# LarsDoorenbos/ccdm-stochastic-segmentation

Hardware: AMD Instinct MI355X
Metric: segmentation samples/sec, LIDC 128x128 T=250 (higher is better)
Workload: dtype f32 (conv products as split fp16 hi/lo x3 on MFMA, fp32 accumulate)

## Files before the change

### ccdm_stochastic_segmentation_amd/csrc/ccdm_attn_block.hip

```cpp
#include "ccdm_common.h"
#include "ccdm_conv_common.h"

namespace ccdm {

struct AttnBlockK {
    ccdm_attn_block_args a;
    const float* wsq;
};

__device__ __forceinline__ void split8(const float* v, f16x8& hi, f16x8& lo) {
#pragma unroll
    for (int j = 0; j < 8; ++j) {
        hi[j] = (_Float16)v[j];
        lo[j] = (_Float16)(v[j] - (float)hi[j]);
    }
}
__device__ __forceinline__ void split4v(const float a, const float b, const float c, const float d, f16x4& hi, f16x4& lo) {
    hi[0] = (_Float16)a; hi[1] = (_Float16)b; hi[2] = (_Float16)c; hi[3] = (_Float16)d;
    lo[0] = (_Float16)(a - (float)hi[0]); lo[1] = (_Float16)(b - (float)hi[1]);
    lo[2] = (_Float16)(c - (float)hi[2]); lo[3] = (_Float16)(d - (float)hi[3]);
}
__device__ __forceinline__ f32x16 mfma3(const f16x8 ah, const f16x8 al, const f16x8 bh, const f16x8 bl, f32x16 acc) {
    acc = __builtin_amdgcn_mfma_f32_32x32x16_f16(al, bh, acc, 0, 0, 0);
    acc = __builtin_amdgcn_mfma_f32_32x32x16_f16(ah, bl, acc, 0, 0, 0);
// ... 171 lines not shown
#pragma unroll
        for (int u = 0; u < 2; ++u)
#pragma unroll
            for (int r = 0; r < 16; ++r) mx = fmaxf(mx, sc[u][r]);
        mx = fmaxf(mx, __shfl_xor(mx, 32));
        const float corr = __expf(m - mx);
        m = mx;
        l *= corr;
#pragma unroll
        for (int r = 0; r < 16; ++r) oo[r] *= corr;
#pragma unroll
        for (int u = 0; u < 2; ++u) {
            float p[16];
#pragma unroll
            for (int r = 0; r < 16; ++r) { p[r] = __expf(sc[u][r] - mx); l += p[r]; }
            const char* vr = vbase + qi * VROW + 2 * ((kt + u) * 32 + 4 * half);
#pragma unroll
            for (int s = 0; s < 2; ++s) {
                f16x8 ph, pl;
                split8(p + 8 * s, ph, pl);
                const f16x8 vh = cat4(*reinterpret_cast<const f16x4*>(vr + 32 * s), *reinterpret_cast<const f16x4*>(vr + 32 * s + 16));
                const f16x8 vl = cat4(*reinterpret_cast<const f16x4*>(vr + 2 * T + 32 * s), *reinterpret_cast<const f16x4*>(vr + 2 * T + 32 * s + 16));
                oo = mfma3(vh, vl, ph, pl, oo);
            }
        }
    }
    l += __shfl_xor(l, 32);
    const float inv = 1.0f / l;
    float* dst = a.out + ((size_t)n * T + mt * 32 + qi) * C + hd * 32 + 4 * half;
#pragma unroll
    for (int g4 = 0; g4 < 4; ++g4) {
        f32x4 v;
#pragma unroll
        for (int e = 0; e < 4; ++e) v[e] = oo[4 * g4 + e] * inv;
        *reinterpret_cast<f32x4*>(dst + 8 * g4) = v;
    }
}

template <int T, int C>
static int launch_one(const AttnBlockK& k, hipStream_t s) {
    using Geo = QkvAttnGeo<T, C>;
    static_assert(Geo::LDS <= 160 * 1024, "LDS budget");
    auto kern = k_qkv_attention<T, C>;
    static bool configured = false;
    if (!configured) {
        if (hipFuncSetAttribute(reinterpret_cast<const void*>(kern), hipFuncAttributeMaxDynamicSharedMemorySize, Geo::LDS) != hipSuccess)
            return fail("norm_qkv_attention: cannot reserve %d bytes of LDS", Geo::LDS);
        configured = true;
    }
    hipLaunchKernelGGL(kern, dim3(k.a.N, k.a.heads), dim3(Geo::NT), Geo::LDS, s, k);
    return 0;
}

bool attn_block_supported(int T, int C, int heads) {
    if (C != heads * 32) return false;
    return (T == 256 && (C == 96 || C == 128)) || (T == 64 && (C == 96 || C == 128)) || (T == 128 && (C == 128 || C == 256));
}

int launch_attn_block(const ccdm_attn_block_args& a, hipStream_t s) {
    CCDM_REQUIRE(a.x && a.out && a.stats && a.gamma && a.beta && a.wqkv && a.bqkv, "norm_qkv_attention: null pointer");
    CCDM_REQUIRE(a.N > 0 && a.slices >= 1, "norm_qkv_attention: N=%d slices=%d", a.N, a.slices);
    {
        int ntiles, NI;
        conv_ntiles(3 * a.C, &ntiles, &NI);
        CCDM_REQUIRE(ntiles == 3 * a.heads, "norm_qkv_attention: packed qkv weights have %d n-tiles, expected %d", ntiles, 3 * a.heads);
    }
    CCDM_REQUIRE(attn_block_supported(a.T, a.C, a.heads), "norm_qkv_attention: (T=%d, C=%d, heads=%d) is not built; use ccdm_conv2d (GN + qkv) + ccdm_attention",
                 a.T, a.C, a.heads);
    AttnBlockK k;
    k.a = a;
    k.wsq = reinterpret_cast<const float*>(static_cast<const char*>(a.wqkv) + (size_t)(a.C / 16) * (3 * a.C / 32) * 2048);
    int rc;
    if (a.T == 256 && a.C == 96) rc = launch_one<256, 96>(k, s);
    else if (a.T == 256) rc = launch_one<256, 128>(k, s);
    else if (a.T == 64 && a.C == 96) rc = launch_one<64, 96>(k, s);
    else if (a.T == 64) rc = launch_one<64, 128>(k, s);
    else if (a.C == 128) rc = launch_one<128, 128>(k, s);
    else rc = launch_one<128, 256>(k, s);
    if (rc) return rc;
    CCDM_CHECK_LAUNCH("norm_qkv_attention");
    return 0;
}

}

extern "C" int ccdm_norm_qkv_attention_supported(int T, int C, int heads) { return ccdm::attn_block_supported(T, C, heads) ? 1 : 0; }

extern "C" int ccdm_norm_qkv_attention(const ccdm_attn_block_args* a, void* stream) {
    if (!a) return ccdm::fail("ccdm_norm_qkv_attention: null args");
    return ccdm::launch_attn_block(*a, (hipStream_t)stream);
}
```

### ccdm_stochastic_segmentation_amd/csrc/ccdm_common.h

```cpp
#pragma once
#include <cstdlib>
#include <hip/hip_runtime.h>
#include <stdint.h>
#include <stdio.h>
#include <string>

#include "ccdm_hip.h"

namespace ccdm {

typedef float f32x16 __attribute__((ext_vector_type(16)));
typedef float f32x4 __attribute__((ext_vector_type(4)));
typedef _Float16 f16x8 __attribute__((ext_vector_type(8)));
typedef _Float16 f16x4 __attribute__((ext_vector_type(4)));

void set_error(const std::string& s);
int fail(const char* fmt, ...);

#define CCDM_CHECK_LAUNCH(what)                                               \
    do {                                                                      \
        hipError_t _e = hipGetLastError();                                    \
        if (_e != hipSuccess) return ::ccdm::fail("%s: %s", what, hipGetErrorString(_e)); \
    } while (0)

#define CCDM_REQUIRE(cond, ...)                     \
    do {                                            \
        if (!(cond)) return ::ccdm::fail(__VA_ARGS__); \
    } while (0)

static inline int cdiv(int a, int b) { return (a + b - 1) / b; }


#ifdef __HIPCC__
template <int BYTES>
__device__ __forceinline__ void warm_kernargs() {
    const auto kp = __builtin_amdgcn_kernarg_segment_ptr();
    static_assert(BYTES <= 512, "eight lines");
    constexpr int L = (BYTES + 63) / 64;
    unsigned d0, d1, d2, d3, d4, d5, d6, d7;
    asm volatile("s_load_dword %0, %8, %9\n\ts_load_dword %1, %8, %10\n\ts_load_dword %2, %8, %11\n\ts_load_dword %3, %8, %12\n\t"
                 "s_load_dword %4, %8, %13\n\ts_load_dword %5, %8, %14\n\ts_load_dword %6, %8, %15\n\ts_load_dword %7, %8, %16\n\t"
                 "s_waitcnt lgkmcnt(0)"
                 : "=&s"(d0), "=&s"(d1), "=&s"(d2), "=&s"(d3), "=&s"(d4), "=&s"(d5), "=&s"(d6), "=&s"(d7)
                 : "s"(kp), "i"(0), "i"(L > 1 ? 0x40 : 0), "i"(L > 2 ? 0x80 : 0), "i"(L > 3 ? 0xc0 : 0), "i"(L > 4 ? 0x100 : 0),
                   "i"(L > 5 ? 0x140 : 0), "i"(L > 6 ? 0x180 : 0), "i"(L > 7 ? 0x1c0 : 0));
}
#endif

struct ConvGeo {
    int TH, TW, waves, MI;
};
static inline ConvGeo conv_geo(int Hout, int Wout, int stride, bool up2 = false, bool fine = false) {
    if (up2) return Wout >= 16 ? ConvGeo{8, 16, 4, 1} : ConvGeo{8, 8, 2, 1};
    if (stride == 2) return Wout >= 16 ? ConvGeo{8, 16, 4, 1} : ConvGeo{8, 8, 2, 1};
    const int area = Hout * Wout;
    if (fine && area <= 1024) return Wout >= 16 && area > 256 ? ConvGeo{8, 16, 4, 1} : ConvGeo{8, 8, 2, 1};
    if (Wout >= 32 && area > 512) return {8, 32, 4, 2};
    if (Wout >= 16 && area > 128) return {8, 16, 4, 1};
    return {8, 8, 2, 1};
}
static inline void conv_ntiles(int Cout, int* ntiles_padded, int* NI) {
    int raw = cdiv(Cout, 32);
    if (raw <= 4) { *NI = raw; *ntiles_padded = raw; return; }
    for (int ni = 4; ni >= 2; --ni)
        if (raw % ni == 0) { *NI = ni; *ntiles_padded = raw; return; }
    *NI = 4; *ntiles_padded = cdiv(raw, 4) * 4;
}
static inline int conv_cin_pad(int Cin) { return cdiv(Cin, 32) * 32; }

int launch_conv(const ccdm_conv_args& a, hipStream_t s);
int launch_conv_input_absmax(const ccdm_conv_args& a, float* out, hipStream_t s);
int launch_attention(const float* qkv, float* out, int N, int T, int Ta, int C, int heads, int order, hipStream_t s);
int launch_posterior(const ccdm_post_args& a, hipStream_t s);
int launch_stats_fold(const double* in, int N, int S_in, int C, int S_out, double* out, hipStream_t s);
int launch_attn_block(const ccdm_attn_block_args& a, hipStream_t s);
int launch_resample(const ccdm_resample_args& a, hipStream_t s);
int launch_stem(const ccdm_stem_args& a, hipStream_t s);
int launch_head(const ccdm_head_args& a, const ccdm_post_args& post, hipStream_t s);
bool attn_block_supported(int T, int C, int heads);

}
```

### ccdm_stochastic_segmentation_amd/csrc/ccdm_conv.hip

```cpp
#include "ccdm_common.h"
#include "ccdm_conv_common.h"

#include <cmath>
#include <cstdlib>
#include <type_traits>
#include <vector>

namespace ccdm {


constexpr int min_waves(int mi, int ni, int prec, int ckt, int threads) {
    if (threads > 512) return 3;
    if (prec != CCDM_PREC_F32 && ckt >= 32) return 2;
    return mi * ni <= 2 ? 3 : (mi * ni <= 4 ? 2 : 1);
}

template <int PREC, int CKT, int KS, int STRIDE, int TH, int TW, int WAVES, int MI, int NI, int KSP = 1, bool UP2 = false, bool SKWT = false>
__global__ __launch_bounds__(WAVES * KSP * 64, min_waves(MI, NI, PREC, CKT, WAVES * KSP * 64)) void k_conv(const ConvK k) {
    constexpr int NT = WAVES * KSP * 64;
    static_assert(KSP == 1 || KSP == KS, "tap split is by kernel row");
    static_assert(!UP2 || (KS == 3 && STRIDE == 1 && KSP == 1 && (NI == 1 || NI == 4) && PREC != CCDM_PREC_F32), "sub-pixel form: 3x3, stride 1, F16X3, one phase or all four");
    constexpr int NTAP = UP2 ? 4 : KS * KS;
    constexpr int CK = CKT, PIXB = conv_pixb(PREC, CKT);
    constexpr int KST = CK / 16;
// ... 852 lines not shown
    ConvK k;
    k.a = a;
    k.core_unmasked = 0;
    const int prec = a.prec & 255;
    k.cin_pad = cin_pad_for(C, prec);
    k.cin_pad_skip = a.skip0 ? cin_pad_for(a.SC0 + a.SC1, prec) : 0;
    k.skip_wide = 0;
    int NI;
    conv_ntiles(up2 ? 4 * a.Cout : a.Cout, &k.ntiles, &NI);
    const int tH = up2 ? a.Hin : a.Hout, tW = up2 ? a.Win : a.Wout;
    const ConvGeo g = conv_geo(tH, tW, a.stride, up2, a.fine_slices != 0);
    if (up2) NI = g.TW == 16 ? 4 : 1;
    else if (g.TW < 32) NI = 1;
    else {
        const long blocks2 = (long)a.N * conv_slices(a.Hout, a.Wout, a.stride, false, a.fine_slices) * (k.ntiles / 2);
        NI = (k.ntiles % 2 == 0 && blocks2 >= 512) ? 2 : 1;
    }
    k.tiles_x = cdiv(tW, g.TW);
    k.tiles_y = cdiv(tH, g.TH);
    k.slices = conv_slices(tH, tW, a.stride, up2, a.fine_slices);
    const bool ks = conv_takes_ks(a);
    if (ks) k.slices = conv_ks_slices(a);
    k.wscale = reinterpret_cast<const float*>(static_cast<const char*>(a.w) +
                                              (up2 ? packed_frag_bytes(4 * a.Cout, C, 2, prec) : packed_frag_bytes(a.Cout, C, a.ksize, prec)));
    const int want_slices = (up2 && NI == 1 ? 4 : 1) * k.slices;
    if (a.out_stats) CCDM_REQUIRE(a.out_slices == want_slices, "conv: out_slices %d != %d", a.out_slices, want_slices);
    if (up2 && upconv_eligible(a)) {
        const int rcu = launch_upconv(a, k.slices, k.ntiles, k.wscale, s);
        if (rcu) return rcu;
        CCDM_CHECK_LAUNCH("upconv");
        return 0;
    }
    if (conv1x1_eligible(a, k.slices)) {
        const int rc1 = launch_conv1x1(a, k.slices, k.ntiles, k.wscale, s);
        if (rc1) return rc1;
        CCDM_CHECK_LAUNCH("conv1x1");
        return 0;
    }
    if (ks) {
        const int rck = launch_conv_ks(a, k.ntiles, k.wscale, s);
        if (rck) return rck;
        CCDM_CHECK_LAUNCH("conv_ks");
        return 0;
    }
    const int HP = ((g.TH - 1) * a.stride + a.ksize) * ((g.TW - 1) * a.stride + a.ksize);
    const int ck = chunk_ck(a, g);
    {
        k.skip_wide = (a.skip0 && prec == CCDM_PREC_F16X3 && a.ksize == 3 && a.stride == 1 && !a.up && g.TW == 32 && NI == 1 && ck == 16 &&
                       a.SC0 % 32 == 0 && a.SC1 % 32 == 0 && !(a.prec >> 8)) ? 1 : 0;
    }
    {
        const int SC = a.SC0 + a.SC1;
        const bool chan_ok = a.C0 % ck == 0 && a.C1 % ck == 0 && (!a.skip0 || (a.SC0 % ck == 0 && a.SC1 % ck == 0 && SC > 0));
        k.core_unmasked = ((up2 ? a.Win : Wc) % (g.TW * a.stride) == 0 && chan_ok) ? 1 : 0;
    }
    CCDM_REQUIRE(a.C1 == 0 || a.C0 % ck == 0, "conv: first source has %d channels; a concatenated input must split at a multiple of the %d-channel chunk", a.C0, ck);
    CCDM_REQUIRE(a.SC1 == 0 || a.SC0 % ck == 0, "conv: first skip source has %d channels; a concatenated input must split at a multiple of the %d-channel chunk", a.SC0, ck);
    CCDM_REQUIRE((k.cin_pad + k.cin_pad_skip) / ck <= 64, "conv: %d input (+%d skip) channels make more than 64 chunks of %d (chunk descriptors live in the 64 lanes of a register)",
                 k.cin_pad, k.cin_pad_skip, ck);
    size_t lds = (size_t)HP * conv_pixb(prec, ck);
    lds = (lds + 15) / 16 * 16;
    if (prec != CCDM_PREC_F32) lds += (size_t)(up2 ? 4 : a.ksize * a.ksize) * (ck / 16) * NI * FRAG_BYTES;
    const int ksp = tap_split(a, g) ? 3 : 1;
    const size_t red = (size_t)g.waves * ksp * NI * 32 * 16;
    if (lds < red) lds = red;
    const size_t epi = (size_t)g.waves * ksp * g.MI * 32 * EPI_ROW * 4;
    if (lds < epi) lds = epi;
    if (a.stats0) {
        const size_t nthreads = (size_t)g.waves * ksp * 64;
        const size_t ex = (size_t)C > nthreads ? (size_t)C : nthreads;
        if (lds < ex * 16) lds = ex * 16;
        lds += (size_t)C * 8;
    }
    CCDM_REQUIRE(lds <= 160 * 1024, "conv: LDS %zu too large", lds);
    dim3 grid(a.N * k.slices, k.ntiles / NI);
    const int rc = prec == CCDM_PREC_F32 ? launch_prec<CCDM_PREC_F32>(k, g, NI, ck, grid, lds, s)
                   : prec == CCDM_PREC_F16 ? launch_prec<CCDM_PREC_F16>(k, g, NI, ck, grid, lds, s)
                                           : launch_prec<CCDM_PREC_F16X3>(k, g, NI, ck, grid, lds, s);
    if (rc) return rc;
    CCDM_CHECK_LAUNCH("conv");
    return 0;
}

}

extern "C" int ccdm_conv_slices(int Hout, int Wout, int stride, int ksize) {
    (void)ksize;
    return ccdm::conv_slices(Hout, Wout, stride);
}

extern "C" int ccdm_upconv_supported(int Cin, int Cout, int prec) {
    return prec == CCDM_PREC_F16X3 && Cin > 0 && Cin % 4 == 0 && Cout > 0 && Cout % 32 == 0;
}

extern "C" int ccdm_upconv_slices(int Hin, int Win) {
    return ccdm::upconv_out_slices(Hin, Win, 0);
}

extern "C" int ccdm_conv_out_slices(const ccdm_conv_args* a) {
    if (!a) return ccdm::fail("ccdm_conv_out_slices: null args");
    return ccdm::conv_out_slices(*a);
}

extern "C" int ccdm_conv_slices_ex(int Hin, int Win, int ksize, int stride, int up, int fine) {
    if (up == 2) return ccdm::upconv_out_slices(Hin, Win, fine);
    const int Hc = up ? 2 * Hin : Hin, Wc = up ? 2 * Win : Win, pad = ksize / 2;
    return ccdm::conv_slices((Hc + 2 * pad - ksize) / stride + 1, (Wc + 2 * pad - ksize) / stride + 1, stride, false, fine);
}

extern "C" int ccdm_conv2d(const ccdm_conv_args* a, void* stream) {
    if (!a) return ccdm::fail("ccdm_conv2d: null args");
    return ccdm::launch_conv(*a, (hipStream_t)stream);
}

extern "C" size_t ccdm_pack_conv_weight_ex(const float* oihw, int Cout, int Cin, int ksize, int prec, const float* cout_absmax, void* out);

extern "C" size_t ccdm_pack_conv_weight(const float* oihw, int Cout, int Cin, int ksize, int prec, void* out) {
    return ccdm_pack_conv_weight_ex(oihw, Cout, Cin, ksize, prec, nullptr, out);
}

extern "C" size_t ccdm_pack_conv_weight_ex(const float* oihw, int Cout, int Cin, int ksize, int prec, const float* cout_absmax, void* out) {
    if (prec != CCDM_PREC_F32 && prec != CCDM_PREC_F16X3) { ccdm::fail("pack: precision %d not built", prec); return 0; }
    int ntiles, NI;
    ccdm::conv_ntiles(Cout, &ntiles, &NI);
    const int cin_pad = ccdm::cin_pad_for(Cin, prec), taps = ksize * ksize;
    const size_t frag = ccdm::packed_frag_bytes(Cout, Cin, ksize, prec);
    const size_t total = frag + (prec == CCDM_PREC_F16X3 ? (size_t)ntiles * 32 * sizeof(float) : 0);
    if (!out) return total;
    if (prec == CCDM_PREC_F32) {
        float* o = static_cast<float*>(out);
        for (int tap = 0; tap < taps; ++tap)
            for (int kp = 0; kp < cin_pad / 2; ++kp)
                for (int nt = 0; nt < ntiles; ++nt)
                    for (int l = 0; l < 64; ++l) {
                        const int co = nt * 32 + (l & 31), ci = 2 * kp + (l >> 5);
                        float v = 0.f;
                        if (co < Cout && ci < Cin) v = oihw[((size_t)co * Cin + ci) * taps + tap];
                        o[(((size_t)tap * (cin_pad / 2) + kp) * ntiles + nt) * 64 + l] = v;
                    }
        return total;
    }
    _Float16* o = static_cast<_Float16*>(out);
    float* sc = reinterpret_cast<float*>(static_cast<char*>(out) + frag);
    std::vector<float> mul(ntiles * 32, 1.0f);
    for (int co = 0; co < ntiles * 32; ++co) {
        float mx = 0.f;
        if (co < Cout) {
            if (cout_absmax) mx = cout_absmax[co];
            else for (size_t i = 0; i < (size_t)Cin * taps; ++i) mx = fmaxf(mx, fabsf(oihw[(size_t)co * Cin * taps + i]));
        }
        int e = 0;
        if (mx > 0.f && std::isfinite(mx)) { int ex; frexpf(mx, &ex); e = 10 - ex; }
        if (e > 60) e = 60;
        if (e < -60) e = -60;
        mul[co] = ldexpf(1.0f, e);
        sc[co] = ldexpf(1.0f, -e) / ccdm::ACT_PRESCALE;
    }
    for (int tap = 0; tap < taps; ++tap)
        for (int ks = 0; ks < cin_pad / 16; ++ks)
            for (int nt = 0; nt < ntiles; ++nt)
                for (int l = 0; l < 64; ++l)
                    for (int j = 0; j < 8; ++j) {
                        const int co = nt * 32 + (l & 31), ci = 16 * ks + 8 * (l >> 5) + j;
                        float v = 0.f;
                        if (co < Cout && ci < Cin) v = oihw[((size_t)co * Cin + ci) * taps + tap] * mul[co];
                        const _Float16 hi = (_Float16)v;
// ... 28 lines not shown
```

### ccdm_stochastic_segmentation_amd/csrc/ccdm_engine.hip

```cpp
#include "ccdm_common.h"

#include <map>
#include <vector>

namespace ccdm {

__global__ void k_step_set(int32_t* p, int32_t v) { *p = v; }
__global__ void k_step_inc(int32_t* p) { *p += 1; }
__global__ void k_run_set(ccdm_post_run* dst, const ccdm_post_run v) { *dst = v; }
__global__ __launch_bounds__(256) void k_absmax(const float* __restrict__ x, size_t n4, float* out) {
    float m = 0.f;
    bool bad = false;
    for (size_t i = (size_t)blockIdx.x * blockDim.x + threadIdx.x; i < n4; i += (size_t)gridDim.x * blockDim.x) {
        const float4 v = reinterpret_cast<const float4*>(x)[i];
        bad |= !(fabsf(v.x) <= 3.0e38f) | !(fabsf(v.y) <= 3.0e38f) | !(fabsf(v.z) <= 3.0e38f) | !(fabsf(v.w) <= 3.0e38f);
        m = fmaxf(m, fmaxf(fmaxf(fabsf(v.x), fabsf(v.y)), fmaxf(fabsf(v.z), fabsf(v.w))));
    }
    if (bad) m = __builtin_inff();
#pragma unroll
    for (int off = 32; off > 0; off >>= 1) m = fmaxf(m, __shfl_xor(m, off));
    if ((threadIdx.x & 63) == 0) atomicMax(reinterpret_cast<unsigned*>(out), __float_as_uint(m));
}

struct Op {
    int kind;
    ccdm_conv_args conv;
    const float* qkv; float* out; int N, T, C, heads, order;
    const double* fin; double* fout; int S_in, S_out;
    ccdm_attn_block_args ab;
    ccdm_resample_args rs;
    ccdm_stem_args st;
    ccdm_head_args hd;
};

static int launch_op(const Op& op, hipStream_t s) {
    switch (op.kind) {
        case 6: return fail("engine: the head + epilogue op is launched with the epilogue's arguments");
        case 0: return launch_conv(op.conv, s);
        case 1: return launch_attention(op.qkv, op.out, op.N, op.T, op.T, op.C, op.heads, op.order, s);
        case 2: return launch_stats_fold(op.fin, op.N, op.S_in, op.C, op.S_out, op.fout, s);
        case 3: return launch_attn_block(op.ab, s);
        case 4: return launch_resample(op.rs, s);
        default: return launch_stem(op.st, s);
    }
}

}

struct ccdm_engine {
    int32_t* step = nullptr;
    std::vector<ccdm::Op> ops;
    ccdm_post_args post{};
    bool has_post = false;
    ccdm_post_run run{};
    ccdm_post_run* run_dev = nullptr;
    bool run_dirty = false;
    int next_row = 0;
    hipGraph_t graph = nullptr;
    hipGraphExec_t exec = nullptr;
    bool graph_valid = false;
    int graph_with_epilogue = -1;
    int captures = 0;
    struct Tap { std::vector<hipEvent_t> ev; int n = 0; };
    std::map<int, Tap> taps;
};

using namespace ccdm;

static void drop_graph(ccdm_engine* e) {
    if (e->exec) { (void)hipGraphExecDestroy(e->exec); e->exec = nullptr; }
    if (e->graph) { (void)hipGraphDestroy(e->graph); e->graph = nullptr; }
    e->graph_valid = false;
}

static int launch_step(ccdm_engine* e, int with_epilogue, hipStream_t s, bool profile) {
    for (size_t i = 0; i < e->ops.size(); ++i) {
        const Op& op = e->ops[i];
        ccdm_engine::Tap* tp = nullptr;
        if (profile) {
            auto it = e->taps.find((int)i);
            if (it != e->taps.end() && (size_t)(2 * it->second.n + 1) < it->second.ev.size()) tp = &it->second;
        }
        if (tp) (void)hipEventRecord(tp->ev[2 * tp->n], s);
        int rc;
        if (op.kind == 6) {
            rc = (with_epilogue && e->has_post) ? launch_head(op.hd, e->post, s) : fail("engine_run: this step ends in a fused head + epilogue op: with_epilogue must be 1 and an epilogue set");
        } else rc = launch_op(op, s);
        if (tp) { (void)hipEventRecord(tp->ev[2 * tp->n + 1], s); tp->n++; }
        if (rc) return rc;
    }
    if (with_epilogue && e->has_post && !(e->ops.size() && e->ops.back().kind == 6)) {
        int rc = launch_posterior(e->post, s);
        if (rc) return rc;
    }
    hipLaunchKernelGGL(k_step_inc, dim3(1), dim3(1), 0, s, e->step);
    CCDM_CHECK_LAUNCH("step_inc");
    return 0;
}

extern "C" ccdm_engine* ccdm_engine_create(int32_t* step_counter) {
    if (!step_counter) { fail("engine_create: null step counter"); return nullptr; }
    ccdm_engine* e = new ccdm_engine();
    e->step = step_counter;
    return e;
}

extern "C" void ccdm_engine_destroy(ccdm_engine* e) {
    if (!e) return;
    drop_graph(e);
    for (auto& kv : e->taps)
        for (hipEvent_t ev : kv.second.ev) (void)hipEventDestroy(ev);
    delete e;
}

extern "C" int ccdm_engine_add_conv(ccdm_engine* e, const ccdm_conv_args* a) {
    CCDM_REQUIRE(e && a, "engine_add_conv: null");
    Op op{};
    op.kind = 0;
    op.conv = *a;
    op.conv.step_ptr = e->step;
    e->ops.push_back(op);
    drop_graph(e);
    return (int)e->ops.size() - 1;
}

extern "C" int ccdm_engine_add_attention(ccdm_engine* e, const float* qkv, float* out, int N, int T, int C, int heads, int order) {
    CCDM_REQUIRE(e && qkv && out, "engine_add_attention: null");
    Op op{};
    op.kind = 1;
    op.qkv = qkv; op.out = out; op.N = N; op.T = T; op.C = C; op.heads = heads; op.order = order;
    e->ops.push_back(op);
    drop_graph(e);
    return (int)e->ops.size() - 1;
}

extern "C" int ccdm_engine_add_norm_qkv_attention(ccdm_engine* e, const ccdm_attn_block_args* a) {
    CCDM_REQUIRE(e && a, "engine_add_norm_qkv_attention: null");
    CCDM_REQUIRE(attn_block_supported(a->T, a->C, a->heads), "engine_add_norm_qkv_attention: (T=%d, C=%d, heads=%d) is not built", a->T, a->C, a->heads);
    Op op{};
    op.kind = 3;
    op.ab = *a;
    e->ops.push_back(op);
    drop_graph(e);
    return (int)e->ops.size() - 1;
}

extern "C" int ccdm_engine_add_stats_fold(ccdm_engine* e, const double* in, int N, int S_in, int C, int S_out, double* out) {
    CCDM_REQUIRE(e && in && out, "engine_add_stats_fold: null");
    Op op{};
    op.kind = 2;
    op.fin = in; op.fout = out; op.N = N; op.S_in = S_in; op.C = C; op.S_out = S_out;
    e->ops.push_back(op);
    drop_graph(e);
    return (int)e->ops.size() - 1;
}

extern "C" int ccdm_engine_add_resample(ccdm_engine* e, const ccdm_resample_args* a) {
    CCDM_REQUIRE(e && a, "engine_add_resample: null");
    Op op{};
    op.kind = 4;
    op.rs = *a;
    e->ops.push_back(op);
    drop_graph(e);
    return (int)e->ops.size() - 1;
}

extern "C" int ccdm_engine_add_stem(ccdm_engine* e, const ccdm_stem_args* a) {
    CCDM_REQUIRE(e && a, "engine_add_stem: null");
    CCDM_REQUIRE(ccdm_stem_conv_supported(a->Cs, a->Cout, a->H, a->W, CCDM_PREC_F16X3), "engine_add_stem: Cs=%d Cout=%d %dx%d is not built", a->Cs, a->Cout, a->H, a->W);
    Op op{};
    op.kind = 5;
    op.st = *a;
    e->ops.push_back(op);
    drop_graph(e);
    return (int)e->ops.size() - 1;
}

extern "C" int ccdm_engine_add_head_posterior(ccdm_engine* e, const ccdm_head_args* a) {
    CCDM_REQUIRE(e && a, "engine_add_head_posterior: null");
    CCDM_REQUIRE(ccdm_head_posterior_supported(a->C, a->K, a->H, a->W, CCDM_PREC_F16X3), "engine_add_head_posterior: C=%d K=%d %dx%d is not built", a->C, a->K, a->H, a->W);
    Op op{};
    op.kind = 6;
    op.hd = *a;
    e->ops.push_back(op);
    drop_graph(e);
    return (int)e->ops.size() - 1;
}

extern "C" int ccdm_engine_set_epilogue(ccdm_engine* e, const ccdm_post_args* a) {
    CCDM_REQUIRE(e && a, "engine_set_epilogue: null");
    e->post = *a;
    e->post.step_ptr = e->step;
    e->has_post = true;
    if (e->run_dev) {
        e->post.run = e->run_dev;
        const ccdm_post_args& p = e->post;
        e->run = ccdm_post_run{p.noise, p.noise_step_stride, p.philox_seed, p.sample_offset, p.noise_row0, p.out_probs, p.out_onehot, p.posterior_out};
        e->run_dirty = true;
    }
    drop_graph(e);
    return 0;
}

extern "C" int ccdm_engine_num_ops(const ccdm_engine* e) { return e ? (int)e->ops.size() : -1; }
extern "C" int ccdm_engine_num_captures(const ccdm_engine* e) { return e ? e->captures : -1; }

extern "C" int ccdm_engine_set_run_block(ccdm_engine* e, void* dev_block) {
    CCDM_REQUIRE(e && e->has_post, "engine_set_run_block: no epilogue set");
    CCDM_REQUIRE(dev_block && (reinterpret_cast<uintptr_t>(dev_block) & 7) == 0, "engine_set_run_block: null or misaligned block");
    e->run_dev = static_cast<ccdm_post_run*>(dev_block);
    e->post.run = e->run_dev;
    const ccdm_post_args& p = e->post;
    e->run = ccdm_post_run{p.noise, p.noise_step_stride, p.philox_seed, p.sample_offset, p.noise_row0, p.out_probs, p.out_onehot, p.posterior_out};
    e->run_dirty = true;
    drop_graph(e);
    return 0;
}

extern "C" int ccdm_engine_set_run(ccdm_engine* e, const float* noise, int64_t noise_step_stride, int32_t noise_row0, uint64_t philox_seed,
                                   uint32_t sample_offset, float* out_probs, int64_t* out_onehot, float* posterior_out) {
    CCDM_REQUIRE(e && e->has_post, "engine_set_run: no epilogue set");
    if (e->run_dev) {
        const ccdm_post_run r{noise, noise_step_stride, philox_seed, sample_offset, noise_row0, out_probs, out_onehot, posterior_out};
        const ccdm_post_run& o = e->run;
        const bool same = o.noise == r.noise && o.noise_step_stride == r.noise_step_stride && o.philox_seed == r.philox_seed &&
                          o.sample_offset == r.sample_offset && o.noise_row0 == r.noise_row0 && o.out_probs == r.out_probs &&
                          o.out_onehot == r.out_onehot && o.posterior_out == r.posterior_out;
        if (!same) { e->run = r; e->run_dirty = true; }
        return 0;
    }
    ccdm_post_args& p = e->post;
    const bool same = p.noise == noise && p.noise_step_stride == noise_step_stride && p.noise_row0 == noise_row0 && p.philox_seed == philox_seed &&
                      p.sample_offset == sample_offset && p.out_probs == out_probs && p.out_onehot == out_onehot &&
                      p.posterior_out == posterior_out;
    if (!same) drop_graph(e);
    p.noise = noise; p.noise_step_stride = noise_step_stride; p.noise_row0 = noise_row0; p.philox_seed = philox_seed; p.sample_offset = sample_offset;
    p.out_probs = out_probs; p.out_onehot = out_onehot; p.posterior_out = posterior_out;
    return 0;
}

extern "C" int ccdm_engine_run(ccdm_engine* e, int first_row, int n_steps, int with_epilogue, int use_graph, void* stream) {
    CCDM_REQUIRE(e, "engine_run: null engine");
    CCDM_REQUIRE(n_steps >= 0, "engine_run: n_steps=%d", n_steps);
    hipStream_t s = (hipStream_t)stream;
    hipLaunchKernelGGL(k_step_set, dim3(1), dim3(1), 0, s, e->step, (int32_t)first_row);
    CCDM_CHECK_LAUNCH("step_set");
    e->next_row = first_row + n_steps;
    if (e->run_dev && e->run_dirty) {
        hipLaunchKernelGGL(k_run_set, dim3(1), dim3(1), 0, s, e->run_dev, e->run);
        CCDM_CHECK_LAUNCH("run_set");
        e->run_dirty = false;
    }
    const bool profile = !e->taps.empty();
    if (profile) {
        use_graph = 0;
        if (first_row == 0) for (auto& kv : e->taps) kv.second.n = 0;
    }
    if (use_graph) {
        if (!e->graph_valid || e->graph_with_epilogue != with_epilogue) {
            drop_graph(e);
            hipError_t err = hipStreamBeginCapture(s, hipStreamCaptureModeRelaxed);
            if (err != hipSuccess) return fail("engine_run: BeginCapture: %s", hipGetErrorString(err));
            const int rc = launch_step(e, with_epilogue, s, false);
            err = hipStreamEndCapture(s, &e->graph);
            if (rc) { if (e->graph) { (void)hipGraphDestroy(e->graph); e->graph = nullptr; } return rc; }
            if (err != hipSuccess) return fail("engine_run: EndCapture: %s", hipGetErrorString(err));
            err = hipGraphInstantiate(&e->exec, e->graph, nullptr, nullptr, 0);
            if (err != hipSuccess) return fail("engine_run: GraphInstantiate: %s", hipGetErrorString(err));
            e->graph_valid = true;
            e->graph_with_epilogue = with_epilogue;
            e->captures++;
        }
        for (int i = 0; i < n_steps; ++i) {
            hipError_t err = hipGraphLaunch(e->exec, s);
            if (err != hipSuccess) return fail("engine_run: GraphLaunch: %s", hipGetErrorString(err));
        }
        return 0;
    }
    for (int i = 0; i < n_steps; ++i) {
        int rc = launch_step(e, with_epilogue, s, profile);
        if (rc) return rc;
    }
    return 0;
}

extern "C" int ccdm_engine_profile_op(ccdm_engine* e, int op_index, int capacity) {
    CCDM_REQUIRE(e, "engine_profile_op: null engine");
    if (op_index < 0) {
        for (auto& kv : e->taps)
            for (hipEvent_t ev : kv.second.ev) (void)hipEventDestroy(ev);
        e->taps.clear();
        return 0;
    }
    CCDM_REQUIRE(op_index < (int)e->ops.size(), "engine_profile_op: op %d out of range", op_index);
    ccdm_engine::Tap& t = e->taps[op_index];
    t.n = 0;
    while ((int)t.ev.size() < 2 * capacity) {
        hipEvent_t ev;
        if (hipEventCreate(&ev) != hipSuccess) return fail("engine_profile_op: hipEventCreate failed");
        t.ev.push_back(ev);
    }
    return 0;
}

extern "C" int ccdm_engine_profile_read(ccdm_engine* e, int op_index, double* mean_ms, double* min_ms, double* max_ms) {
    CCDM_REQUIRE(e, "engine_profile_read: null engine");
    auto it = e->taps.find(op_index);
    CCDM_REQUIRE(it != e->taps.end(), "engine_profile_read: op %d is not tapped", op_index);
    ccdm_engine::Tap& t = it->second;
    double sum = 0, mn = 1e30, mx = 0;
    int n = 0;
    for (int i = 0; i < t.n; ++i) {
        float ms = 0.f;
        if (hipEventSynchronize(t.ev[2 * i + 1]) != hipSuccess) continue;
        if (hipEventElapsedTime(&ms, t.ev[2 * i], t.ev[2 * i + 1]) != hipSuccess) continue;
        sum += ms; if (ms < mn) mn = ms; if (ms > mx) mx = ms; ++n;
    }
    if (mean_ms) *mean_ms = n ? sum / n : 0.0;
    if (min_ms) *min_ms = n ? mn : 0.0;
    if (max_ms) *max_ms = n ? mx : 0.0;
    return n;
}

extern "C" int ccdm_engine_input_absmax(ccdm_engine* e, float* out, int row, void* stream) {
    CCDM_REQUIRE(e && out, "engine_input_absmax: null");
    hipStream_t s = (hipStream_t)stream;
    const int r = row >= 0 ? row : (e->next_row > 0 ? e->next_row - 1 : 0);
    hipLaunchKernelGGL(k_step_set, dim3(1), dim3(1), 0, s, e->step, (int32_t)r);
    CCDM_CHECK_LAUNCH("step_set");
    int rc = 0;
    for (size_t i = 0; i < e->ops.size() && !rc; ++i) {
        const Op& op = e->ops[i];
        if (op.kind == 0) rc = launch_conv_input_absmax(op.conv, out + i, s);
        else if (op.kind == 6) {
            ccdm_conv_args c{};
            c.in0 = op.hd.x; c.C0 = op.hd.C; c.stats0 = op.hd.stats; c.slices0 = op.hd.slices; c.gamma = op.hd.gamma; c.beta = op.hd.beta;
            c.eps = op.hd.eps; c.act = CCDM_ACT_SILU; c.N = op.hd.N; c.Hin = c.Hout = op.hd.H; c.Win = c.Wout = op.hd.W; c.ksize = 3; c.stride = 1;
            c.emb_off = -1; c.prec = CCDM_PREC_F16X3;
            rc = launch_conv_input_absmax(c, out + i, s);
        }
        else if (op.kind == 5 || op.kind == 1) {
            const size_t n4 = op.kind == 5 ? (size_t)op.st.N * op.st.H * op.st.W * op.st.Cs / 4 : (size_t)op.N * op.T * 3 * op.C / 4;
            const float* src = op.kind == 5 ? op.st.xin : op.qkv;
            const unsigned bx = (unsigned)(n4 / 256 < 1 ? 1 : (n4 / 256 > 1024 ? 1024 : n4 / 256));
            hipLaunchKernelGGL(k_absmax, dim3(bx), dim3(256), 0, s, src, n4, out + i);
            if (hipGetLastError() != hipSuccess) rc = fail("engine_input_absmax: attention operand probe failed to launch");
        }
    }
    hipLaunchKernelGGL(k_step_set, dim3(1), dim3(1), 0, s, e->step, (int32_t)e->next_row);
    CCDM_CHECK_LAUNCH("step_set");
    return rc;
}

extern "C" int ccdm_engine_describe_op(const ccdm_engine* e, int i, char* buf, int buflen) {
    CCDM_REQUIRE(e && buf && buflen > 0, "engine_describe_op: bad args");
    CCDM_REQUIRE(i >= 0 && i < (int)e->ops.size(), "engine_describe_op: op %d out of range", i);
    const Op& op = e->ops[i];
    if (op.kind == 0) {
        const ccdm_conv_args& a = op.conv;
        snprintf(buf, buflen, "conv%dx%d %d%s->%d in%dx%d out%dx%d s%d%s%s%s%s%s%s", a.ksize, a.ksize, a.C0 + a.C1,
                 a.C1 ? "(cat)" : "", a.Cout, a.Hin, a.Win, a.Hout, a.Wout, a.stride, a.up ? " up2x" : "",
                 a.stats0 ? " gn" : "", a.act ? " silu" : "", a.emb_off >= 0 ? " +emb" : "", a.resid ? " +res" : "",
                 a.out_stats ? " stats" : "");
    } else if (op.kind == 1) {
        snprintf(buf, buflen, "attention T=%d C=%d heads=%d order=%d", op.T, op.C, op.heads, op.order);
// ... 15 lines not shown
```

### ccdm_stochastic_segmentation_amd/csrc/ccdm_misc.hip

```cpp
#include "ccdm_common.h"

#include <stdarg.h>

namespace ccdm {

static thread_local std::string g_err;
void set_error(const std::string& s) { g_err = s; }
int fail(const char* fmt, ...) {
    char buf[512];
    va_list ap;
    va_start(ap, fmt);
    vsnprintf(buf, sizeof buf, fmt, ap);
    va_end(ap);
    g_err = buf;
    return -1;
}

__global__ void k_gn_stats(const float* __restrict__ x, int HW, int C, int slices, double* __restrict__ stats) {
    extern __shared__ __attribute__((aligned(16))) char smem[];
    double* red = reinterpret_cast<double*>(smem);
    const int Q = C >> 2, R = blockDim.x / Q;
    const int q = threadIdx.x % Q, r = threadIdx.x / Q;
    const int s = blockIdx.x, n = blockIdx.y;
    const int p0 = (int)((long long)HW * s / slices), p1 = (int)((long long)HW * (s + 1) / slices);
// ... 48 lines not shown
    float m = -INFINITY, l = 0.f;

    for (int j0 = 0; j0 < T; j0 += 64) {
        __syncthreads();
        for (int item = lane; item < 64 * (D / 4); item += 64) {
            const int row = item / (D / 4), c4 = item % (D / 4);
            float4 kv = make_float4(0, 0, 0, 0), vv = make_float4(0, 0, 0, 0);
            if (j0 + row < T) {
                const float* p = base + (size_t)(j0 + row) * C3;
                kv = *reinterpret_cast<const float4*>(p + koff + 4 * c4);
                vv = *reinterpret_cast<const float4*>(p + voff + 4 * c4);
            }
            kv.x *= scale; kv.y *= scale; kv.z *= scale; kv.w *= scale;
            *reinterpret_cast<float4*>(kt + row * D + 4 * c4) = kv;
            *reinterpret_cast<float4*>(vt + row * D + 4 * c4) = vv;
        }
        __syncthreads();
        const int jn = (T - j0) < 64 ? (T - j0) : 64;
        for (int jb = 0; jb < jn; jb += 16) {
            float s[16];
            float mx = m;
#pragma unroll
            for (int jj = 0; jj < 16; ++jj) {
                const float* kr = kt + (jb + jj) * D;
                float acc = 0.f;
#pragma unroll
                for (int c = 0; c < D; ++c) acc = fmaf(q[c], kr[c], acc);
                s[jj] = (jb + jj < jn) ? acc : -INFINITY;
                mx = fmaxf(mx, s[jj]);
            }
            const float corr = expf(m - mx);
            l *= corr;
#pragma unroll
            for (int c = 0; c < D; ++c) o[c] *= corr;
            m = mx;
#pragma unroll
            for (int jj = 0; jj < 16; ++jj) {
                const float p = expf(s[jj] - mx);
                l += p;
                const float* vr = vt + (jb + jj) * D;
#pragma unroll
                for (int c = 0; c < D; ++c) o[c] = fmaf(p, vr[c], o[c]);
            }
        }
    }
    if (t < T) {
        const float inv = 1.0f / l;
        float* dst = out + ((size_t)n * Ta + t) * C + h * D;
#pragma unroll
        for (int c = 0; c < D; c += 4)
            *reinterpret_cast<float4*>(dst + c) = make_float4(o[c] * inv, o[c + 1] * inv, o[c + 2] * inv, o[c + 3] * inv);
    }
}

int launch_attention_mfma(const float* qkv, float* out, int N, int T, int Ta, int C, int heads, int order, hipStream_t s);
int attention_mfma_width(int D);

int launch_attention(const float* qkv, float* out, int N, int T, int Ta, int C, int heads, int order, hipStream_t s) {
    CCDM_REQUIRE(qkv && out, "attention: null pointer");
    CCDM_REQUIRE(heads > 0 && C % heads == 0, "attention: C=%d not divisible by heads=%d", C, heads);
    CCDM_REQUIRE(T > 0 && Ta >= T, "attention: T=%d, %d rows allocated per sample", T, Ta);
    const int D = C / heads;
    const bool force_valu = (order & CCDM_ATTENTION_FORCE_VALU) != 0;
    order &= 255;
    const bool mfma_ok = attention_mfma_width(D) > 0 && !(D == 32 && (T % 32 != 0 || Ta != T));
    if (mfma_ok && !force_valu) return launch_attention_mfma(qkv, out, N, T, Ta, C, heads, order, s);
    dim3 grid(cdiv(T, 64), heads, N), block(64);
    switch (D) {
        case 4: hipLaunchKernelGGL(k_attention<4>, grid, block, 0, s, qkv, out, T, Ta, C, heads, order); break;
        case 8: hipLaunchKernelGGL(k_attention<8>, grid, block, 0, s, qkv, out, T, Ta, C, heads, order); break;
        case 12: hipLaunchKernelGGL(k_attention<12>, grid, block, 0, s, qkv, out, T, Ta, C, heads, order); break;
        case 16: hipLaunchKernelGGL(k_attention<16>, grid, block, 0, s, qkv, out, T, Ta, C, heads, order); break;
        case 24: hipLaunchKernelGGL(k_attention<24>, grid, block, 0, s, qkv, out, T, Ta, C, heads, order); break;
        case 32: hipLaunchKernelGGL(k_attention<32>, grid, block, 0, s, qkv, out, T, Ta, C, heads, order); break;
        case 48: hipLaunchKernelGGL(k_attention<48>, grid, block, 0, s, qkv, out, T, Ta, C, heads, order); break;
        case 64: hipLaunchKernelGGL(k_attention<64>, grid, block, 0, s, qkv, out, T, Ta, C, heads, order); break;
        default: return fail("attention: head width %d (C=%d / heads=%d) is built neither on the matrix cores (multiples of 4 up to 128) nor "
                             "on the vector path (4, 8, 12, 16, 24, 32, 48, 64): choose num_heads / num_head_channels accordingly", D, C, heads);
    }
    CCDM_CHECK_LAUNCH("attention");
    return 0;
}

__device__ __forceinline__ float silu_t(float x) { return x / (1.0f + expf(-x)); }

__global__ void k_time_table(const float* __restrict__ sinus, int mc,
                             const float* __restrict__ w0, const float* __restrict__ b0,
                             const float* __restrict__ w2, const float* __restrict__ b2,
                             const float* __restrict__ wcat, const float* __restrict__ bcat, int E,
                             float* __restrict__ emb_out, float* __restrict__ out) {
    extern __shared__ __attribute__((aligned(16))) float sm[];
    const int ted = 4 * mc;
    float* x = sm;
    float* h1 = sm + mc;
    float* e = h1 + ted;
    const int s = blockIdx.x;
    for (int i = threadIdx.x; i < mc; i += blockDim.x) x[i] = sinus[(size_t)s * mc + i];
    __syncthreads();
    for (int j = threadIdx.x; j < ted; j += blockDim.x) {
        float acc = 0.f;
        for (int i = 0; i < mc; ++i) acc = fmaf(w0[(size_t)j * mc + i], x[i], acc);
        h1[j] = silu_t(acc + b0[j]);
    }
    __syncthreads();
    for (int j = threadIdx.x; j < ted; j += blockDim.x) {
        float acc = 0.f;
        for (int i = 0; i < ted; ++i) acc = fmaf(w2[(size_t)j * ted + i], h1[i], acc);
        const float v = acc + b2[j];
        if (emb_out) emb_out[(size_t)s * ted + j] = v;
        e[j] = silu_t(v);
    }
    __syncthreads();
    for (int j = threadIdx.x; j < E; j += blockDim.x) {
        float acc = 0.f;
        for (int i = 0; i < ted; ++i) acc = fmaf(wcat[(size_t)j * ted + i], e[i], acc);
        out[(size_t)s * E + j] = acc + bcat[j];
    }
}

__global__ void k_nchw_to_nhwc(const float* __restrict__ src, float* __restrict__ dst, int C, int HW,
                               int dst_stride, int dst_off, size_t total) {
    const size_t i = (size_t)blockIdx.x * blockDim.x + threadIdx.x;
    if (i >= total) return;
    const int p = (int)(i % HW);
    const size_t nc = i / HW;
    const int c = (int)(nc % C);
    const size_t n = nc / C;
    dst[(n * HW + p) * dst_stride + dst_off + c] = src[i];
}

__global__ void k_onehot_to_xin(const uint8_t* __restrict__ idx, float* __restrict__ xin, int K, int stride, size_t npix) {
    const size_t i = (size_t)blockIdx.x * blockDim.x + threadIdx.x;
    if (i >= npix) return;
    const int k = idx[i];
    float* d = xin + i * stride;
    for (int c = 0; c < K; ++c) d[c] = (c == k) ? 1.0f : 0.0f;
}

}

using namespace ccdm;

extern "C" int ccdm_version(void) { return CCDM_ABI_VERSION; }
extern "C" const char* ccdm_last_error_string(void) { return g_err.c_str(); }

namespace ccdm {
__global__ void k_stats_fold(const double* __restrict__ in, int S_in, int C2, int S_out, double* __restrict__ out) {
    const int n = blockIdx.y;
    const int i = blockIdx.x * blockDim.x + threadIdx.x;
    if (i >= S_out * C2) return;
    const int j = i / C2, c = i % C2;
    const int s0 = (int)((long long)j * S_in / S_out), s1 = (int)((long long)(j + 1) * S_in / S_out);
    const double* p = in + (size_t)n * S_in * C2 + c;
    double t = 0.0;
    for (int s = s0; s < s1; s += 16) {
        double v[16];
#pragma unroll
        for (int u = 0; u < 16; ++u) v[u] = p[(size_t)min(s + u, s1 - 1) * C2];
#pragma unroll
        for (int u = 0; u < 16; ++u) t += s + u < s1 ? v[u] : 0.0;
    }
    out[(size_t)n * S_out * C2 + i] = t;
}
int launch_stats_fold(const double* in, int N, int S_in, int C, int S_out, double* out, hipStream_t s) {
    CCDM_REQUIRE(in && out && N > 0 && C > 0, "stats_fold: bad arguments");
    CCDM_REQUIRE(S_out >= 1 && S_out <= CCDM_STATS_MAX_SLICES && S_in >= S_out, "stats_fold: %d -> %d slices", S_in, S_out);
    dim3 grid((unsigned)cdiv(S_out * C * 2, 256), (unsigned)N);
    hipLaunchKernelGGL(k_stats_fold, grid, dim3(256), 0, s, in, S_in, 2 * C, S_out, out);
    CCDM_CHECK_LAUNCH("stats_fold");
    return 0;
}
}

extern "C" int ccdm_stats_fold(const double* in, int N, int S_in, int C, int S_out, double* out, void* stream) {
    return ccdm::launch_stats_fold(in, N, S_in, C, S_out, out, (hipStream_t)stream);
}

extern "C" int ccdm_gn_stats(const float* x, int N, int HW, int C, int slices, double* stats, void* stream) {
    CCDM_REQUIRE(x && stats, "gn_stats: null pointer");
    CCDM_REQUIRE(C % 4 == 0 && C >= 4 && C <= 1024, "gn_stats: C=%d must be a multiple of 4 in [4,1024]", C);
    CCDM_REQUIRE(slices >= 1 && slices <= CCDM_STATS_MAX_SLICES, "gn_stats: slices=%d", slices);
    const int Q = C / 4;
    const int R = 256 / Q > 0 ? 256 / Q : 1;
    dim3 grid(slices, N), block(Q * R);
    const size_t lds = (size_t)Q * R * 8 * sizeof(double);
    hipLaunchKernelGGL(k_gn_stats, grid, block, lds, (hipStream_t)stream, x, HW, C, slices, stats);
    CCDM_CHECK_LAUNCH("gn_stats");
    return 0;
}

extern "C" int ccdm_attention(const float* qkv, float* out, int N, int T, int C, int heads, int order, void* stream) {
    return launch_attention(qkv, out, N, T, T, C, heads, order, (hipStream_t)stream);
}

extern "C" int ccdm_time_table(const float* sinus, int S, int mc, const float* w0, const float* b0,
                               const float* w2, const float* b2, const float* wcat, const float* bcat, int E,
                               float* emb_out, float* out, void* stream) {
    CCDM_REQUIRE(sinus && w0 && b0 && w2 && b2 && out, "time_table: null pointer");
    CCDM_REQUIRE(E == 0 || (wcat && bcat), "time_table: null wcat/bcat");
    CCDM_REQUIRE(mc > 0 && mc <= 1024, "time_table: model_channels=%d", mc);
    if (S <= 0) return 0;
    const size_t lds = (size_t)(mc + 8 * mc) * sizeof(float);
    hipLaunchKernelGGL(k_time_table, dim3(S), dim3(256), lds, (hipStream_t)stream, sinus, mc, w0, b0, w2, b2,
                       wcat, bcat, E, emb_out, out);
    CCDM_CHECK_LAUNCH("time_table");
    return 0;
}

extern "C" int ccdm_nchw_to_nhwc(const float* src, float* dst, int N, int C, int HW, int dst_stride, int dst_off, void* stream) {
    CCDM_REQUIRE(src && dst, "nchw_to_nhwc: null pointer");
    const size_t total = (size_t)N * C * HW;
    if (!total) return 0;
    hipLaunchKernelGGL(k_nchw_to_nhwc, dim3((unsigned)((total + 255) / 256)), dim3(256), 0, (hipStream_t)stream,
                       src, dst, C, HW, dst_stride, dst_off, total);
    CCDM_CHECK_LAUNCH("nchw_to_nhwc");
    return 0;
}

extern "C" int ccdm_onehot_to_xin(const uint8_t* idx, float* xin, int N, int HW, int K, int xin_stride, void* stream) {
    CCDM_REQUIRE(idx && xin, "onehot_to_xin: null pointer");
    const size_t npix = (size_t)N * HW;
    if (!npix) return 0;
    hipLaunchKernelGGL(k_onehot_to_xin, dim3((unsigned)((npix + 255) / 256)), dim3(256), 0, (hipStream_t)stream,
                       idx, xin, K, xin_stride, npix);
    CCDM_CHECK_LAUNCH("onehot_to_xin");
    return 0;
}


namespace ccdm {

constexpr int LN_MAX_PER_LANE = 24;
__global__ __launch_bounds__(256) void k_layernorm(const float* __restrict__ x, const float* __restrict__ gamma, const float* __restrict__ beta,
                                                   float eps, long rows, int C, float* __restrict__ out) {
    const long row = (long)blockIdx.x * 4 + (threadIdx.x >> 6);
    const int lane = threadIdx.x & 63;
    if (row >= rows) return;
    const float* xr = x + row * C;
    float v[LN_MAX_PER_LANE];
    float sum = 0.f;
#pragma unroll
    for (int i = 0; i < LN_MAX_PER_LANE; ++i) {
        const int c = lane + 64 * i;
        v[i] = c < C ? xr[c] : 0.f;
        sum += v[i];
    }
#pragma unroll
    for (int off = 32; off > 0; off >>= 1) sum += __shfl_xor(sum, off);
    const float mean = sum / (float)C;
    float dsum = 0.f;
#pragma unroll
    for (int i = 0; i < LN_MAX_PER_LANE; ++i) {
        const int c = lane + 64 * i;
// ... 122 lines not shown
```

### ccdm_stochastic_segmentation_amd/csrc/ccdm_resample.hip

```cpp
#include "ccdm_common.h"
#include "ccdm_conv_common.h"

namespace ccdm {

struct ResampleK {
    ccdm_conv_args g;
    float* out_act;
    float* out_raw;
    int mode;
};

__device__ __forceinline__ float4 resample_act(const float4 v, const float2* ab, const int c, const bool has_gn, const bool silu) {
    float x[4] = {v.x, v.y, v.z, v.w};
#pragma unroll
    for (int j = 0; j < 4; ++j) {
        float y = x[j];
        if (has_gn) y = fmaf(y, ab[c + j].x, ab[c + j].y);
        if (silu) y = y / (1.0f + expf(-y));
        x[j] = y;
    }
    return make_float4(x[0], x[1], x[2], x[3]);
}

__device__ __forceinline__ float4 pool4(const float4 a, const float4 b, const float4 c, const float4 d) {
    return make_float4((((a.x + b.x) + c.x) + d.x) * 0.25f, (((a.y + b.y) + c.y) + d.y) * 0.25f,
                       (((a.z + b.z) + c.z) + d.z) * 0.25f, (((a.w + b.w) + c.w) + d.w) * 0.25f);
}

__global__ __launch_bounds__(256) void k_resample(const ResampleK k) {
    extern __shared__ __attribute__((aligned(16))) char smem_rs[];
    float2* ab = reinterpret_cast<float2*>(smem_rs);
    const ccdm_conv_args& a = k.g;
    const int n = blockIdx.y, C = a.C0, Q = C >> 2;
    const bool has_gn = a.stats0 != nullptr && k.out_act != nullptr, silu = a.act == CCDM_ACT_SILU;
    if (has_gn) {
        compute_gn_affine(a, n, 0, ab);
        __syncthreads();
    }
    const int Ho = a.Hout, Wo = a.Wout;
    const float* in = a.in0 + (size_t)n * a.Hin * a.Win * C;
    float* oa = k.out_act ? k.out_act + (size_t)n * Ho * Wo * C : nullptr;
    float* orw = k.out_raw ? k.out_raw + (size_t)n * Ho * Wo * C : nullptr;
    const long long items = (long long)Ho * Wo * Q;
    for (long long item = (long long)blockIdx.x * blockDim.x + threadIdx.x; item < items; item += (long long)gridDim.x * blockDim.x) {
        const int q = (int)(item % Q), p = (int)(item / Q), ox = p % Wo, oy = p / Wo, c = 4 * q;
        const size_t o = (size_t)p * C + c;
        if (k.mode == CCDM_RESAMPLE_AVGPOOL2) {
            const float* r0 = in + ((size_t)(2 * oy) * a.Win + 2 * ox) * C + c;
            const float* r1 = r0 + (size_t)a.Win * C;
            const float4 v00 = *reinterpret_cast<const float4*>(r0), v01 = *reinterpret_cast<const float4*>(r0 + C);
            const float4 v10 = *reinterpret_cast<const float4*>(r1), v11 = *reinterpret_cast<const float4*>(r1 + C);
            if (orw) *reinterpret_cast<float4*>(orw + o) = pool4(v00, v01, v10, v11);
            if (oa)
                *reinterpret_cast<float4*>(oa + o) = pool4(resample_act(v00, ab, c, has_gn, silu), resample_act(v01, ab, c, has_gn, silu),
                                                           resample_act(v10, ab, c, has_gn, silu), resample_act(v11, ab, c, has_gn, silu));
        } else {
            const float4 v = *reinterpret_cast<const float4*>(in + ((size_t)(oy >> 1) * a.Win + (ox >> 1)) * C + c);
            if (orw) *reinterpret_cast<float4*>(orw + o) = v;
            if (oa) *reinterpret_cast<float4*>(oa + o) = resample_act(v, ab, c, has_gn, silu);
        }
    }
}

int launch_resample(const ccdm_resample_args& r, hipStream_t s) {
    CCDM_REQUIRE(r.in && (r.out_act || r.out_raw), "resample: null pointer");
    CCDM_REQUIRE(r.mode == CCDM_RESAMPLE_AVGPOOL2 || r.mode == CCDM_RESAMPLE_NEAREST_UP2, "resample: mode = %d", r.mode);
    CCDM_REQUIRE(r.C > 0 && r.C % 4 == 0 && r.N > 0 && r.Hin > 0 && r.Win > 0, "resample: N=%d C=%d %dx%d", r.N, r.C, r.Hin, r.Win);
    CCDM_REQUIRE(r.act == CCDM_ACT_NONE || r.act == CCDM_ACT_SILU, "resample: act = %d", r.act);
    ResampleK k{};
    k.g.in0 = r.in; k.g.C0 = r.C;
    k.g.N = r.N; k.g.Hin = r.Hin; k.g.Win = r.Win;
    k.g.Hout = r.mode == CCDM_RESAMPLE_AVGPOOL2 ? r.Hin / 2 : 2 * r.Hin;
    k.g.Wout = r.mode == CCDM_RESAMPLE_AVGPOOL2 ? r.Win / 2 : 2 * r.Win;
    CCDM_REQUIRE(k.g.Hout > 0 && k.g.Wout > 0, "resample: AvgPool2d(2) of a %dx%d image is empty", r.Hin, r.Win);
    k.g.act = r.act; k.g.eps = r.eps; k.g.emb_off = -1;
    if (r.stats) {
        CCDM_REQUIRE(r.out_act, "resample: GroupNorm statistics without an out_act destination");
        CCDM_REQUIRE(r.C % 32 == 0 && r.C <= CCDM_MAX_CHANNELS, "resample: GroupNorm(32, %d)", r.C);
        CCDM_REQUIRE(r.gamma && r.beta && r.slices >= 1 && r.slices <= CCDM_STATS_MAX_SLICES, "resample: GroupNorm needs gamma/beta and 1..%d slices (got %d)",
                     CCDM_STATS_MAX_SLICES, r.slices);
        k.g.stats0 = r.stats; k.g.slices0 = r.slices; k.g.gamma = r.gamma; k.g.beta = r.beta;
    }
    k.out_act = r.out_act; k.out_raw = r.out_raw; k.mode = r.mode;
    const long long items = (long long)k.g.Hout * k.g.Wout * (r.C / 4);
    const long long want = (items + 1023) / 1024;
    const int bx = (int)(want < 1 ? 1 : (want > 64 ? 64 : want));
    hipLaunchKernelGGL(k_resample, dim3(bx, r.N), dim3(256), r.stats ? (size_t)r.C * 8 : 0, s, k);
    CCDM_CHECK_LAUNCH("resample");
    return 0;
}

}

extern "C" int ccdm_resample(const ccdm_resample_args* a, void* stream) {
    if (!a) return ccdm::fail("ccdm_resample: null args");
    return ccdm::launch_resample(*a, (hipStream_t)stream);
}
```

### ccdm_stochastic_segmentation_amd/engine.py

```python
from __future__ import annotations

import ctypes as C
import math
from dataclasses import dataclass
from typing import Dict, List, Optional, Sequence, Tuple

import numpy as np
import torch

from . import hip
from .unet_spec import GN_EPS, UNetSpec


@dataclass
class DevTensor:
    buf: torch.Tensor
    C: int
    h: int
    w: int
    stats: Optional[torch.Tensor] = None
    slices: int = 0

    @property
    def ptr(self) -> int:
        return self.buf.data_ptr()

    @property
    def stats_ptr(self) -> int:
        return self.stats.data_ptr() if self.stats is not None else 0


def timestep_embedding_host(timesteps: torch.Tensor, dim: int, max_period: int = 10000) -> torch.Tensor:
    half = dim // 2
    freqs = torch.exp(-math.log(max_period) * torch.arange(start=0, end=half, dtype=torch.float32) / half)
    args = timesteps[:, None].float() * freqs[None]
    emb = torch.cat([torch.cos(args), torch.sin(args)], dim=-1)
    if dim % 2:
        emb = torch.cat([emb, torch.zeros_like(emb[:, :1])], dim=-1)
    return emb


class TileCanvas:

    def __init__(self, n: int, Hc: int, Wc: int, sy: int, sx: int, K: int, device: torch.device):
        self.n, self.Hc, self.Wc, self.sy, self.sx = int(n), int(Hc), int(Wc), int(sy), int(sx)
        self.xt = torch.zeros((self.n, self.Hc * self.Wc), dtype=torch.uint8, device=device)
        self.out_probs = torch.empty((self.n, self.Hc, self.Wc, K), dtype=torch.float32, device=device)
        self.out_onehot = torch.empty((self.n, self.Hc, self.Wc, K), dtype=torch.int64, device=device)


class SamplerEngine:

    def __init__(self, spec: UNetSpec, state_dict: Dict[str, torch.Tensor], N: int, H: int, W: int,
                 num_classes: int, img_channels: int, device: torch.device, max_steps: int,
                 feature_shape: Optional[Tuple[int, int, int]] = None, prec: int = hip.PREC_F32, fine_slices: int = 0,
                 f32_layers=frozenset()):
        self.lib = hip.load()
        self.f32_layers = frozenset(f32_layers)
        self.fine_slices = int(fine_slices)
        if device.type != "cuda":
            raise hip.CcdmHipError("SamplerEngine needs a HIP device (torch device 'cuda'); there is no CPU path")
        self.spec, self.N, self.H, self.W = spec, int(N), int(H), int(W)
        self.K, self.C_img = int(num_classes), int(img_channels)
        self.device, self.prec = device, prec
        self.max_steps = max(int(max_steps), self.N, 1)
        if spec.in_channels != self.K + self.C_img or spec.out_channels != self.K:
            raise ValueError("spec channels do not match num_classes/img_channels")
        self._keep: List[torch.Tensor] = []
        self._sd = {k: v.detach().to("cpu", torch.float32).contiguous() for k, v in state_dict.items()}
        self.feature_shape = feature_shape
        self._handle = None
        self._tile_canvas: Optional[TileCanvas] = None
        self._tile_canvas_key = None
        self._bound_xt: Optional[torch.Tensor] = None
        self._bound_ws: Optional[torch.Tensor] = None
        self._slot_pools: Optional[Tuple[torch.Tensor, torch.Tensor]] = None
        with torch.cuda.device(device):
            self.stream = torch.cuda.Stream(device=device)
            with torch.cuda.stream(self.stream):
                self._build()
            self.stream.synchronize()

    def _dev(self, shape, dtype=torch.float32, zero=False) -> torch.Tensor:
        t = (torch.zeros if zero else torch.empty)(shape, dtype=dtype, device=self.device)
        self._keep.append(t)
        return t

    def _upload(self, arr) -> torch.Tensor:
        t = torch.as_tensor(np.ascontiguousarray(arr)) if not isinstance(arr, torch.Tensor) else arr.contiguous()
        d = t.to(self.device)
        self._keep.append(d)
        return d

    def _act(self, C_: int, h: int, w: int, stats: bool, slices: int = 0) -> DevTensor:
        buf = self._dev((self.N, h, w, C_))
        t = DevTensor(buf, C_, h, w)
        if stats:
            t.slices = slices
            t.stats = self._dev((self.N, t.slices, C_, 2), torch.float64)
        return t

    def _fold_stats(self, t: DevTensor) -> None:
        if t.stats is None or t.slices <= hip.STATS_MAX_SLICES:
            return
        folded = self._dev((self.N, hip.STATS_FOLD_SLICES, t.C, 2), torch.float64)
        hip.check(self.lib.ccdm_engine_add_stats_fold(self._handle, t.stats.data_ptr(), self.N, t.slices, t.C, hip.STATS_FOLD_SLICES,
                                                      folded.data_ptr()), "engine_add_stats_fold")
        self.op_names.append("stats_fold")
        self.op_info.append(dict(kind="stats_fold", name="stats_fold", io_bytes=0, gn_read_bytes=0, weight_bytes=0, flop=0))
        t.stats, t.slices = folded, hip.STATS_FOLD_SLICES

    def _conv(self, src: Sequence[DevTensor], wkey: str, cout: int, ksize: int, *, gn: Optional[str] = None,
              act: int = hip.ACT_NONE, stride: int = 1, up: bool = False, emb_off: int = -1,
              film_off: int = -1, resid: Optional[DevTensor] = None, stats: bool = True,
              skip_src: Optional[Sequence[DevTensor]] = None, skip_key: Optional[str] = None) -> DevTensor:
        sd = self._sd
        prec = hip.PREC_F32 if wkey in self.f32_layers else self.prec
        pack_prec = hip.PREC_F16X3 if prec == hip.PREC_F16 else prec
        a, b = src[0], (src[1] if len(src) > 1 else None)
        cin = a.C + (b.C if b else 0)
        w = sd[wkey + ".weight"].numpy()
        assert w.shape[0] == cout and w.shape[1] <= cin, (wkey, w.shape, cin, cout)
        if w.shape[1] < cin:
            wp = np.zeros((cout, cin) + tuple(w.shape[2:]), np.float32)
            wp[:, : w.shape[1]] = w
            w = wp
        bias_np = sd[wkey + ".bias"].numpy()
        absmax = None
        if skip_src is not None:
            ws = sd[skip_key + ".weight"].numpy().reshape(cout, -1)
            absmax = np.maximum(np.abs(w.reshape(cout, -1)).max(1), np.abs(ws).max(1)).astype(np.float32)
            skip_w = self._upload(hip.pack_conv_weight(ws.reshape(cout, -1, 1, 1), 1, pack_prec, absmax))
            bias_np = bias_np + sd[skip_key + ".bias"].numpy()
        subpixel = bool(up) and ksize == 3 and stride == 1 and resid is None and skip_src is None and gn is None and emb_off < 0 and \
            bool(self.lib.ccdm_upconv_supported(cin, cout, prec))
        wdev = self._upload(hip.pack_upconv_weight(w, prec) if subpixel else hip.pack_conv_weight(w, ksize, pack_prec, absmax))
        bias = self._upload(bias_np)
        hin, win = a.h, a.w
        hc, wc = (2 * hin, 2 * win) if up else (hin, win)
        pad = ksize // 2
# ... 203 lines not shown
        ted, mc = spec.time_embed_dim, spec.model_channels
        self.emb_offsets: Dict[str, int] = {}
        ws, bs, off = [], [], 0
        for name, l in spec.all_layers():
            if l.kind == "res":
                self.emb_offsets[name] = off
                ws.append(sd[name + ".emb_layers.1.weight"].numpy())
                bs.append(sd[name + ".emb_layers.1.bias"].numpy())
                off += ws[-1].shape[0]
        self.E = off
        self.wcat = self._upload(np.concatenate(ws, 0))
        self.bcat = self._upload(np.concatenate(bs, 0))
        self.te = [self._upload(sd[k].numpy()) for k in
                   ("time_embed.0.weight", "time_embed.0.bias", "time_embed.2.weight", "time_embed.2.bias")]
        S = self.max_steps
        self.sinus = self._dev((S, mc))
        self.emb_table = self._dev((S, self.E))
        self.step_table = self._dev((S, 4), zero=True)

        self.Cs = (K + self.C_img + 3) // 4 * 4
        self.xt = self._dev((N, H * W), torch.uint8, zero=True)
        self.xin = DevTensor(self._dev((N, H, W, self.Cs), zero=True), self.Cs, H, W)
        self.feat: Optional[DevTensor] = None
        if spec.feature_condition_idx:
            if self.feature_shape is None:
                raise ValueError("this model concatenates feature conditioning; feature_shape=(C,h,w) is required")
            fc, fh, fw = self.feature_shape
            if fc != spec.feature_channels:
                raise ValueError(f"feature_condition has {fc} channels, model expects {spec.feature_channels}")
            self.feat = DevTensor(self._dev((N, fh, fw, fc)), fc, fh, fw,
                                  self._dev((N, 1, fc, 2), torch.float64), 1)
        self.out_probs = self._dev((N, H, W, K))
        self.out_onehot = self._dev((N, H, W, K), torch.int64)

        hs: List[DevTensor] = []
        h = self.xin
        for i, blk in enumerate(spec.input_blocks):
            src = [h]
            if i in spec.feature_condition_idx:
                if (self.feat.h, self.feat.w) != (h.h, h.w):
                    raise ValueError(f"feature_condition is {self.feat.h}x{self.feat.w}, U-Net stage is {h.h}x{h.w}")
                src = [h, self.feat]
            h = self._layers(blk, src)
            hs.append(h)
        h = self._layers(spec.middle_block, [h])
        for blk in spec.output_blocks:
            h = self._layers(blk, [h, hs.pop()])
        Kp = (K + 3) // 4 * 4
        if Kp != K:
            wk, bk = self._sd["out.2.weight"], self._sd["out.2.bias"]
            self._sd["out.2.weight"] = torch.cat([wk, torch.zeros((Kp - K,) + tuple(wk.shape[1:]))], 0)
            self._sd["out.2.bias"] = torch.cat([bk, torch.zeros(Kp - K)], 0)
        self.head_fused = bool(self.prec == hip.PREC_F16X3 and "out.2" not in self.f32_layers and not self.fine_slices and h.stats is not None
                               and lib.ccdm_head_posterior_supported(h.C, K, H, W, hip.PREC_F16X3))
        self._head_src = h
        self.head = None if self.head_fused else self._conv([h], "out.2", Kp, 3, gn="out.0", act=hip.ACT_SILU, stats=False)
        self.head_ce: Optional[DevTensor] = None
        if spec.ce_head:
            Kc = K - 1
            Kcp = (Kc + 3) // 4 * 4
            if Kcp != Kc:
                wk, bk = self._sd["out_ce.2.weight"], self._sd["out_ce.2.bias"]
                self._sd["out_ce.2.weight"] = torch.cat([wk, torch.zeros((Kcp - Kc,) + tuple(wk.shape[1:]))], 0)
                self._sd["out_ce.2.bias"] = torch.cat([bk, torch.zeros(Kcp - Kc)], 0)
            self.head_ce = self._conv([h], "out_ce.2", Kcp, 3, gn="out_ce.0", act=hip.ACT_SILU, stats=False)
        if self.head_fused:
            sdw = self._sd
            a = hip.HeadArgs()
            a.x, a.stats, a.slices = h.ptr, h.stats_ptr, h.slices
            a.gamma = self._upload(sdw["out.0.weight"].numpy()).data_ptr()
            a.beta = self._upload(sdw["out.0.bias"].numpy()).data_ptr()
            a.eps = GN_EPS
            a.w = self._upload(hip.pack_head_weight(sdw["out.2.weight"].numpy()[:K])).data_ptr()
            a.bias = self._upload(sdw["out.2.bias"].numpy()[:K]).data_ptr()
            a.N, a.H, a.W, a.C, a.K = N, H, W, h.C, K
            a.logits_out = 0
            hip.check(lib.ccdm_engine_add_head_posterior(self._handle, C.byref(a)), "engine_add_head_posterior")
            self.op_names.append("out.2")
            self.op_info.append(dict(kind="conv", name="out.2", cin=h.C, cout=Kp, k=3, hin=H, win=W, hout=H, wout=W, stride=1, up=False,
                                     subpixel=False, gn=True, skip=False, prec=hip.PREC_F16X3, skip_wide=False, head_fused=True,
                                     io_bytes=4 * (h.C * H * W + Kp * H * W), gn_read_bytes=4 * h.C * H * W, weight_bytes=4 * Kp * h.C * 9,
                                     flop=2 * h.C * Kp * 9 * H * W))
        self.n_unet_ops = lib.ccdm_engine_num_ops(self._handle)

        post = hip.PostArgs()
        post.head, post.softmax, post.head_stride = (0 if self.head_fused else self.head.ptr), int(spec.softmax_output), (Kp if self.head_fused else self.head.C)
        post.xt, post.N, post.HW, post.K = self.xt.data_ptr(), N, H * W, K
        post.step_table, post.step_ptr = self.step_table.data_ptr(), 0
        post.noise, post.noise_step_stride = 0, 0
        post.philox_seed, post.sample_offset = 0, 0
        post.xt_next = self.xt.data_ptr()
        post.xin, post.xin_stride = (0 if self.stem_onehot_on_load else self.xin.ptr), self.Cs
        post.out_probs, post.out_onehot, post.posterior_out = self.out_probs.data_ptr(), self.out_onehot.data_ptr(), 0
        self.flag = self._dev((1,), torch.int32, zero=True)
        post.noise_row0, post.range_flag = 0, self.flag.data_ptr()
        self._post = post
        hip.check(lib.ccdm_engine_set_epilogue(self._handle, C.byref(post)), "engine_set_epilogue")
        self.run_block = self._dev((hip.POST_RUN_BYTES // 8,), torch.int64, zero=True)
        hip.check(lib.ccdm_engine_set_run_block(self._handle, self.run_block.data_ptr()), "engine_set_run_block")
        self._sd = None
        self._tables_key = None
        self._per_sample_rows = False

    def __del__(self):
        try:
            if self._handle:
                self.lib.ccdm_engine_destroy(self._handle)
                self._handle = None
        except Exception:
            pass

    def _stream(self) -> int:
        return self.stream.cuda_stream

    def enter(self):
        self.stream.wait_stream(torch.cuda.current_stream(self.device))
        return torch.cuda.stream(self.stream)

    def leave(self) -> None:
        torch.cuda.current_stream(self.device).wait_stream(self.stream)

    def graph_captures(self) -> int:
        return int(self.lib.ccdm_engine_num_captures(self._handle))

    def describe_ops(self) -> List[str]:
        out = []
        buf = C.create_string_buffer(256)
        for i in range(self.n_unet_ops):
            self.lib.ccdm_engine_describe_op(self._handle, i, buf, 256)
            out.append(f"{i:3d} {self.op_names[i]}: {buf.value.decode()}")
        return out

    def set_inputs(self, xt_idx: torch.Tensor, cond: torch.Tensor, feat: Optional[torch.Tensor] = None) -> None:
        lib, s, N, HW = self.lib, self._stream(), self.N, self.H * self.W
        assert tuple(xt_idx.shape) == (N, self.H, self.W) and xt_idx.dtype == torch.uint8 and xt_idx.is_cuda
        assert tuple(cond.shape) == (N, self.C_img, self.H, self.W), (tuple(cond.shape), (N, self.C_img, self.H, self.W))
        cond = cond.to(self.device, torch.float32).contiguous()
        self.xt.copy_(xt_idx.reshape(N, HW))
        hip.check(lib.ccdm_nchw_to_nhwc(cond.data_ptr(), self.xin.ptr, N, self.C_img, HW, self.Cs, self.K, s), "nchw_to_nhwc")
        hip.check(lib.ccdm_onehot_to_xin(self.xt.data_ptr(), self.xin.ptr, N, HW, self.K, self.Cs, s), "onehot_to_xin")
        if self.feat is not None:
            if feat is None:
                raise ValueError("feature_condition is required by this model")
            f = self.feat
            assert tuple(feat.shape) == (N, f.C, f.h, f.w), tuple(feat.shape)
            feat = feat.to(self.device, torch.float32).contiguous()
            hip.check(lib.ccdm_nchw_to_nhwc(feat.data_ptr(), f.ptr, N, f.C, f.h * f.w, f.C, 0, s), "nchw_to_nhwc(feat)")
            hip.check(lib.ccdm_gn_stats(f.ptr, N, f.h * f.w, f.C, 1, f.stats_ptr, s), "gn_stats(feat)")
        self._cond_keepalive = (cond, feat)

    def set_slot_inputs(self, n0: int, xt_idx: torch.Tensor, cond: torch.Tensor) -> None:
        lib, s, HW = self.lib, self._stream(), self.H * self.W
        n = int(xt_idx.shape[0])
        n0 = int(n0)
        if self.feat is not None:
            raise ValueError("set_slot_inputs: a model that takes a feature_condition is not built")
        assert 0 <= n0 and n >= 1 and n0 + n <= self.N, (n0, n, self.N)
        assert tuple(xt_idx.shape) == (n, self.H, self.W) and xt_idx.dtype == torch.uint8 and xt_idx.is_cuda and xt_idx.is_contiguous()
        assert tuple(cond.shape) == (n, self.C_img, self.H, self.W) and cond.dtype == torch.float32 and cond.is_cuda and cond.is_contiguous()
        self.xt[n0:n0 + n].copy_(xt_idx.reshape(n, HW))
        xin = self.xin.ptr + n0 * HW * self.Cs * 4
        hip.check(lib.ccdm_nchw_to_nhwc(cond.data_ptr(), xin, n, self.C_img, HW, self.Cs, self.K, s), "nchw_to_nhwc")
        hip.check(lib.ccdm_onehot_to_xin(self.xt.data_ptr() + n0 * HW, xin, n, HW, self.K, self.Cs, s), "onehot_to_xin")

    def set_rows(self, rows: torch.Tensor, non_blocking: bool = False) -> None:
        assert tuple(rows.shape) == (self.N,) and rows.dtype == torch.int32
        self.rowmap.copy_(rows, non_blocking=non_blocking)
        self._tables_key = None

    def slots_step(self, table: torch.Tensor) -> None:
        assert table.is_cuda and table.is_contiguous() and table.numel() * table.element_size() == self.N * C.sizeof(hip.SlotRow)
        hip.check(self.lib.ccdm_slots_step(self.out_probs.data_ptr(), table.data_ptr(), self.N, self.H * self.W, self.K, self.xt.data_ptr(),
                                           None if self.stem_onehot_on_load else self.xin.ptr, self.Cs, self.out_probs.data_ptr(),
                                           self.out_onehot.data_ptr(), self._stream()), "slots_step")

    def _slot_guidance_pools(self) -> Tuple[torch.Tensor, torch.Tensor]:
        if self._slot_pools is None:
            self._slot_pools = (torch.zeros((self.N, self.H * self.W, self.K), dtype=torch.float32, device=self.device),
                                torch.full((self.N, self.H * self.W), 255, dtype=torch.uint8, device=self.device))
        return self._slot_pools

    def set_slot_guidance(self, n0: int, evidence: Optional[torch.Tensor], known: Optional[torch.Tensor]) -> None:
        n0, HW = int(n0), self.H * self.W
        ev_pool, known_pool = self._slot_guidance_pools()
        for name, t, pool, dtype in (("evidence", evidence, ev_pool, torch.float32), ("known", known, known_pool, torch.uint8)):
            if t is None:
                continue
            n = int(t.shape[0])
            assert 0 <= n0 and n >= 1 and n0 + n <= self.N, (name, n0, n, self.N)
            assert tuple(t.shape) == (n, *pool.shape[1:]) and t.dtype == dtype and t.is_cuda and t.is_contiguous(), (name, tuple(t.shape), t.dtype)
            pool[n0:n0 + n].copy_(t)

    def slots_guided_step(self, table: torch.Tensor, guide_table: torch.Tensor) -> None:
        assert table.is_cuda and table.is_contiguous() and table.numel() * table.element_size() == self.N * C.sizeof(hip.SlotRow)
        assert guide_table.is_cuda and guide_table.is_contiguous() and \
            guide_table.numel() * guide_table.element_size() == self.N * C.sizeof(hip.SlotGuideRow)
        ev_pool, known_pool = self._slot_guidance_pools()
        hip.check(self.lib.ccdm_slots_guided_step(self.out_probs.data_ptr(), table.data_ptr(), guide_table.data_ptr(), ev_pool.data_ptr(),
                                                  known_pool.data_ptr(), self.N, self.H * self.W, self.K, self.xt.data_ptr(),
                                                  None if self.stem_onehot_on_load else self.xin.ptr, self.Cs, self.out_probs.data_ptr(),
                                                  self.out_onehot.data_ptr(), self._stream()), "slots_guided_step")

    def _bound_args(self, labels: torch.Tensor, table: torch.Tensor) -> int:
        assert labels.dtype == torch.uint8 and labels.is_cuda and labels.is_contiguous() and labels.dim() == 2 and \
            labels.shape[1] == self.H * self.W, (labels.dtype, tuple(labels.shape))
        assert table.is_cuda and table.is_contiguous() and table.numel() * table.element_size() == self.N * C.sizeof(hip.BoundRow)
        return int(labels.shape[0])

    def bound_noise(self, labels: torch.Tensor, table: torch.Tensor, *, philox_seed: int = 0) -> torch.Tensor:
        R = self._bound_args(labels, table)
        if self._bound_xt is None:
            self._bound_xt = torch.zeros((self.N, self.H, self.W), dtype=torch.uint8, device=self.device)
        hip.check(self.lib.ccdm_bound_noise(labels.data_ptr(), table.data_ptr(), self.N, R, self.H * self.W, self.K,
                                            int(philox_seed) & (2 ** 64 - 1), self._bound_xt.data_ptr(), self._stream()), "bound_noise")
        return self._bound_xt

    def bound_terms(self, labels: torch.Tensor, table: torch.Tensor, weights: Optional[torch.Tensor], floor: float, row_sum: torch.Tensor,
                    row_weight: torch.Tensor, map: Optional[torch.Tensor] = None) -> None:
        R = self._bound_args(labels, table)
        assert weights is None or (weights.dtype == torch.float32 and weights.is_cuda and weights.is_contiguous() and weights.numel() == self.K)
        for v in (row_sum, row_weight):
            assert v.dtype == torch.float64 and v.is_cuda and v.is_contiguous() and v.numel() == self.N
        assert map is None or (map.dtype == torch.float32 and map.is_cuda and map.is_contiguous() and map.numel() == self.N * self.H * self.W)
        if self._bound_ws is None:
            nbytes = int(self.lib.ccdm_bound_terms_workspace_bytes(self.N, self.H * self.W, self.K))
            self._bound_ws = torch.zeros((nbytes // 8,), dtype=torch.float64, device=self.device)
        hip.check(self.lib.ccdm_bound_terms(self.out_probs.data_ptr(), self.xt.data_ptr(), labels.data_ptr(), table.data_ptr(),
                                            None if weights is None else weights.data_ptr(), self.N, R, self.H * self.W, self.K, float(floor),
                                            self._bound_ws.data_ptr(), row_sum.data_ptr(), row_weight.data_ptr(),
                                            None if map is None else map.data_ptr(), self._stream()), "bound_terms")

    def set_tables(self, t_rows: Sequence[float], coeffs: Sequence[Tuple[float, float, int]], per_sample: bool = False) -> None:
        S = len(t_rows)
        if S > self.max_steps:
            raise ValueError(f"{S} table rows > max_steps {self.max_steps}")
        key = (tuple(float(t) for t in t_rows), tuple(coeffs), per_sample)
        if key == self._tables_key:
            return
        sin = timestep_embedding_host(torch.tensor(list(t_rows), dtype=torch.float32), self.spec.model_channels)
        self.sinus[:S].copy_(sin)
        tab = torch.zeros((S, 4), dtype=torch.float32)
        for i, (a, c, mode) in enumerate(coeffs):
            tab[i, 0], tab[i, 1], tab[i, 2] = a, c, float(mode)
        self.step_table[:S].copy_(tab)
        self.rowmap.copy_(torch.arange(self.N, dtype=torch.int32) if per_sample else torch.zeros(self.N, dtype=torch.int32))
        self._per_sample_rows = bool(per_sample)
        w0, b0, w2, b2 = (t.data_ptr() for t in self.te)
        hip.check(self.lib.ccdm_time_table(self.sinus.data_ptr(), S, self.spec.model_channels, w0, b0, w2, b2,
                                           self.wcat.data_ptr(), self.bcat.data_ptr(), self.E, 0,
                                           self.emb_table.data_ptr(), self._stream()), "time_table")
        self._tables_key = key

    def run(self, n_steps: int, *, noise: Optional[torch.Tensor] = None, philox_seed: int = 0, sample_offset: int = 0,
            with_epilogue: bool = True, use_graph: bool = False, first_row: int = 0, noise_row0: int = 0,
            posterior_out: Optional[torch.Tensor] = None) -> None:
        npn = self.N * self.H * self.W * self.K
        if noise is not None:
            assert noise.is_cuda and noise.dtype == torch.float32 and noise.is_contiguous()
            assert first_row >= noise_row0 and noise.numel() >= max(first_row - noise_row0 + n_steps - 1, 1) * npn, "noise tensor too small"
            self._noise_keepalive = noise
        hip.check(self.lib.ccdm_engine_set_run(
            self._handle, noise.data_ptr() if noise is not None else 0, npn, int(noise_row0), int(philox_seed) & (2 ** 64 - 1),
            int(sample_offset), self.out_probs.data_ptr(), self.out_onehot.data_ptr(),
            posterior_out.data_ptr() if posterior_out is not None else 0), "engine_set_run")
        hip.check(self.lib.ccdm_engine_run(self._handle, first_row, n_steps, int(with_epilogue), int(use_graph),
                                           self._stream()), "engine_run")

    def _step_state_args(self, philox_seed: int, sample_offset: int) -> tuple:
        return (int(philox_seed) & (2 ** 64 - 1), int(sample_offset), self.xt.data_ptr(),
                None if self.stem_onehot_on_load else self.xin.ptr, self.Cs)

    def clamp_known_labels(self, known: torch.Tensor, cumalpha_tm1: float, mode: int, step_row: int, *, philox_seed: int = 0,
                           sample_offset: int = 0) -> None:
        assert known.dtype == torch.uint8 and known.is_cuda and known.is_contiguous() and tuple(known.shape) == (self.N, self.H * self.W)
        c = float(cumalpha_tm1)
        p_miss = (1.0 - c) / self.K
        last = mode != hip.STEP_SAMPLE
        hip.check(self.lib.ccdm_known_labels_step(
            known.data_ptr(), self.N, self.H * self.W, self.K, float(np.float32(c + p_miss)), float(np.float32(p_miss)), int(mode),
            int(step_row), *self._step_state_args(philox_seed, sample_offset), self.out_probs.data_ptr() if last else None,
            self.out_onehot.data_ptr() if last else None, self._stream()), "known_labels_step")
        self._known_keepalive = known

    def renoise(self, p_stay: float, p_move: float, step_row: int, *, philox_seed: int = 0, sample_offset: int = 0) -> None:
        hip.check(self.lib.ccdm_renoise_step(
            self.N, self.H * self.W, self.K, float(p_stay), float(p_move), int(step_row), *self._step_state_args(philox_seed, sample_offset),
            self._stream()), "renoise_step")

    def tile_canvas(self, n: int, Hc: int, Wc: int, sy: int, sx: int) -> TileCanvas:
        key = (int(n), int(Hc), int(Wc), int(sy), int(sx))
        if self._tile_canvas_key != key:
            R = (1 + -((self.H - key[1]) // key[3])) * (1 + -((self.W - key[2]) // key[4]))
            if not (1 <= key[3] <= self.H <= key[1] and 1 <= key[4] <= self.W <= key[2]) or R * key[0] != self.N:
                raise ValueError(f"tiles: an engine of {self.N} rows of {self.H}x{self.W} does not hold the tiles of {key[0]} canvases "
                                 f"{key[1]}x{key[2]} at strides ({key[3]}, {key[4]})")
            self._tile_canvas = TileCanvas(*key, self.K, self.device)
            self._tile_canvas_key = key
        return self._tile_canvas

    def guided_step(self, evidence: Optional[torch.Tensor], shaping: Optional[Tuple[float, float]], views: Optional[Sequence[int]],
                    alpha_t: float, cumalpha_tm1: float, mode: int, step_row: int, *, philox_seed: int = 0, sample_offset: int = 0,
                    canvas: Optional[TileCanvas] = None) -> None:
        flips = () if views is None else tuple(int(f) for f in views)
        V = 1 + len(flips)
        if canvas is not None:
            assert views is None and canvas is self._tile_canvas
            n, pixels = canvas.n, canvas.Hc * canvas.Wc
        else:
            assert 1 <= V <= 4 and self.N % V == 0 and all(0 <= f <= 3 for f in flips)
            n, pixels = self.N // V, self.H * self.W
        assert evidence is None or (evidence.dtype == torch.float32 and evidence.is_cuda and evidence.is_contiguous()
                                    and tuple(evidence.shape) == (n, pixels, self.K))
        x0, ev = self.out_probs.data_ptr(), None if evidence is None else evidence.data_ptr()
        inv_t, top_r = (float(v) for v in shaping or (1.0, 1.0))
        seed, off, *state = self._step_state_args(philox_seed, sample_offset)
        step = (float(alpha_t), float(cumalpha_tm1), int(mode), int(step_row), seed, off)
        outputs = self if canvas is None else canvas
        tail = (*state, outputs.out_probs.data_ptr(), outputs.out_onehot.data_ptr(), self._stream())
        if canvas is not None:
            hip.check(self.lib.ccdm_tiled_step(x0, ev, n, canvas.Hc, canvas.Wc, self.H, self.W, canvas.sy, canvas.sx, self.K, inv_t, top_r, *step,
                                               canvas.xt.data_ptr(), *tail), "tiled_step")
        elif views is not None:
            hip.check(self.lib.ccdm_views_step(x0, ev, n, self.H, self.W, self.K, V, sum(f << (2 * (v + 1)) for v, f in enumerate(flips)),
                                               inv_t, top_r, *step, *tail), "views_step")
        elif shaping is not None:
            hip.check(self.lib.ccdm_shaped_step(x0, ev, n, pixels, self.K, inv_t, top_r, *step, *tail), "shaped_step")
        else:
            hip.check(self.lib.ccdm_evidence_step(x0, ev, n, pixels, self.K, *step, *tail), "evidence_step")
        self._evidence_keepalive = evidence

    def ce_logits(self) -> Optional[torch.Tensor]:
        if self.head_ce is None:
            return None
        return self.head_ce.buf[..., : self.K - 1].clone().permute(0, 3, 1, 2)

    def probe_buffer(self) -> torch.Tensor:
        with self.enter():
            buf = torch.zeros((self.n_unet_ops,), dtype=torch.float32, device=self.device)
# ... 48 lines not shown
```

### ccdm_stochastic_segmentation_amd/hip.py

```python
from __future__ import annotations

import ctypes as C
import os
import subprocess
from typing import Optional

_HERE = os.path.dirname(os.path.abspath(__file__))
ROOT = os.path.dirname(_HERE)
LIB_PATH = os.environ.get("CCDM_LIB") or os.path.join(_HERE, "libccdm_hip.so")
CSRC = os.path.join(_HERE, "csrc")
SOURCES = ["ccdm_conv.hip", "ccdm_conv_ks.hip", "ccdm_upconv.hip", "ccdm_stem.hip", "ccdm_head.hip", "ccdm_conv1x1.hip", "ccdm_misc.hip", "ccdm_attention.hip", "ccdm_attn_block.hip", "ccdm_sampler.hip", "ccdm_known.hip", "ccdm_guided.hip", "ccdm_metrics.hip", "ccdm_range.hip", "ccdm_resample.hip", "ccdm_engine.hip", "ccdm_vote.hip", "ccdm_segeval.hip", "ccdm_segexport.hip", "ccdm_csscore.hip", "ccdm_segcalib.hip", "ccdm_segboundary.hip", "ccdm_contourf.hip", "ccdm_uncscore.hip", "ccdm_lidcscore.hip", "ccdm_surfdist.hip", "ccdm_lesions.hip", "ccdm_lesionmatch.hip", "ccdm_findings.hip", "ccdm_modes.hip", "ccdm_bound.hip"]
HIPCC_FLAGS = ["--offload-arch=gfx950", "-O3", "-std=c++17", "-ffp-contract=off", "-mllvm", "-amdgpu-mfma-vgpr-form=1", "-fPIC", "-shared"]

ACT_NONE, ACT_SILU = 0, 1
RESAMPLE_AVGPOOL2, RESAMPLE_NEAREST_UP2 = 0, 1
ATTENTION_FORCE_VALU = 256
ATTENTION_VALU_WIDTHS = (4, 8, 12, 16, 24, 32, 48, 64)
DIAG_GENERAL_KERNEL = 2048 << 8
PREC_F32, PREC_F16X3 = 0, 1
PREC_F16 = 2
STEP_SAMPLE, STEP_LAST_CONFIDENCE, STEP_LAST_MAJORITY, STEP_LAST_KEEP, STEP_SOFTMAX_ONLY = 0, 1, 2, 3, 4
SLOT_IDLE = -1
SLOT_GUIDE_EVIDENCE, SLOT_GUIDE_KNOWN = 1, 2
BOUND_IDLE = -1
# ... 171 lines not shown
                                  C.c_float, C.c_int, C.c_int, C.c_uint64, C.c_uint32, C.c_void_p, C.c_void_p, C.c_int, C.c_void_p, C.c_void_p,
                                  C.c_void_p]),
    "ccdm_tiled_step": (C.c_int, [C.c_void_p, C.c_void_p, C.c_int, C.c_int, C.c_int, C.c_int, C.c_int, C.c_int, C.c_int, C.c_int, C.c_float,
                                  C.c_float, C.c_float, C.c_float, C.c_int, C.c_int, C.c_uint64, C.c_uint32, C.c_void_p, C.c_void_p, C.c_void_p,
                                  C.c_int, C.c_void_p, C.c_void_p, C.c_void_p]),
    "ccdm_slots_step": (C.c_int, [C.c_void_p, C.c_void_p, C.c_int, C.c_int, C.c_int, C.c_void_p, C.c_void_p, C.c_int, C.c_void_p, C.c_void_p,
                                  C.c_void_p]),
    "ccdm_slots_guided_step": (C.c_int, [C.c_void_p, C.c_void_p, C.c_void_p, C.c_void_p, C.c_void_p, C.c_int, C.c_int, C.c_int, C.c_void_p,
                                         C.c_void_p, C.c_int, C.c_void_p, C.c_void_p, C.c_void_p]),
    "ccdm_bound_noise": (C.c_int, [C.c_void_p, C.c_void_p, C.c_int, C.c_int, C.c_int, C.c_int, C.c_uint64, C.c_void_p, C.c_void_p]),
    "ccdm_bound_terms_workspace_bytes": (C.c_size_t, [C.c_int, C.c_int, C.c_int]),
    "ccdm_bound_terms": (C.c_int, [C.c_void_p, C.c_void_p, C.c_void_p, C.c_void_p, C.c_void_p, C.c_int, C.c_int, C.c_int, C.c_int, C.c_float,
                                   C.c_void_p, C.c_void_p, C.c_void_p, C.c_void_p, C.c_void_p]),
    "ccdm_pairwise_class_counts": (C.c_int, [C.c_void_p, C.c_void_p, C.c_int, C.c_int, C.c_int, C.c_int, C.c_int, C.c_void_p, C.c_void_p]),
    "ccdm_lidcscore": (C.c_int, [C.c_void_p, C.c_void_p, C.c_int, C.c_int, C.c_int, C.c_int, C.c_int, C.c_void_p, C.c_void_p, C.c_void_p]),
    "ccdm_surfdist_workspace_bytes": (C.c_size_t, [C.c_int, C.c_int, C.c_int, C.c_int, C.c_int, C.c_int]),
    "ccdm_surfdist": (C.c_int, [C.c_void_p, C.c_void_p, C.c_int, C.c_int, C.c_int, C.c_int, C.c_int, C.c_int, C.c_int, C.c_int, C.c_void_p,
                                C.c_void_p, C.c_void_p, C.c_size_t, C.c_void_p]),
    "ccdm_lesions_workspace_bytes": (C.c_size_t, [C.c_int, C.c_int, C.c_int, C.c_int, C.c_int, C.c_int]),
    "ccdm_lesions": (C.c_int, [C.c_void_p, C.c_void_p, C.c_int, C.c_int, C.c_int, C.c_int, C.c_int, C.c_int, C.c_int, C.c_void_p, C.c_int,
                               C.c_void_p, C.c_void_p, C.c_size_t, C.c_void_p]),
    "ccdm_lesion_match_workspace_bytes": (C.c_size_t, [C.c_int, C.c_int, C.c_int, C.c_int, C.c_int, C.c_int]),
    "ccdm_lesion_match": (C.c_int, [C.c_int, C.c_int, C.c_int, C.c_int, C.c_int, C.c_int, C.c_void_p, C.c_int, C.c_int, C.c_void_p, C.c_void_p,
                                    C.c_void_p, C.c_size_t, C.c_void_p]),
    "ccdm_findings_workspace_bytes": (C.c_size_t, [C.c_int, C.c_int, C.c_int, C.c_int, C.c_int, C.c_int, C.c_int]),
    "ccdm_findings": (C.c_int, [C.c_void_p, C.c_void_p, C.c_int, C.c_int, C.c_int, C.c_int, C.c_int, C.c_int, C.c_int, C.c_int, C.c_int, C.c_int,
                                C.c_void_p, C.c_void_p, C.c_void_p, C.c_void_p, C.c_void_p, C.c_size_t, C.c_void_p]),
    "ccdm_vote_accumulate": (C.c_int, [C.c_void_p, C.c_void_p, C.c_int64, C.c_int, C.c_int, C.c_int, C.c_float, C.c_void_p, C.c_void_p,
                                       C.c_void_p, C.c_void_p]),
    "ccdm_vote_finalize": (C.c_int, [C.c_void_p, C.c_void_p, C.c_void_p, C.c_int, C.c_int, C.c_int, C.c_int, C.c_void_p, C.c_void_p,
                                     C.c_void_p, C.c_void_p, C.c_void_p]),
    "ccdm_vote_reduce_stack": (C.c_int, [C.c_void_p, C.c_int, C.c_int, C.c_int, C.c_int, C.c_void_p, C.c_void_p, C.c_void_p, C.c_void_p,
                                         C.c_void_p]),
    "ccdm_modes_distance": (C.c_int, [C.c_void_p, C.c_int, C.c_int, C.c_int, C.c_int, C.c_void_p, C.c_void_p, C.c_void_p]),
    "ccdm_modes_pam": (C.c_int, [C.c_void_p, C.c_int, C.c_int, C.c_int, C.c_int, C.c_void_p, C.c_void_p, C.c_void_p, C.c_void_p, C.c_void_p,
                                 C.c_void_p, C.c_void_p, C.c_void_p]),
    "ccdm_modes_maps": (C.c_int, [C.c_void_p, C.c_void_p, C.c_void_p, C.c_int, C.c_int, C.c_int, C.c_int, C.c_int, C.c_void_p, C.c_void_p,
                                  C.c_void_p, C.c_void_p]),
    "ccdm_seg_confusion_workspace_bytes": (C.c_size_t, [C.c_int, C.c_int, C.c_int, C.c_int]),
    "ccdm_seg_confusion": (C.c_int, [C.c_void_p, C.c_int64, C.c_void_p, C.c_void_p, C.c_int, C.c_int, C.c_int, C.c_int, C.c_int, C.c_int,
                                     C.c_void_p, C.c_void_p, C.c_void_p, C.c_size_t, C.c_void_p]),
    "ccdm_segexport": (C.c_int, [C.c_void_p, C.c_int64, C.c_void_p, C.c_int, C.c_int, C.c_int, C.c_int, C.c_int, C.c_int, C.c_int,
                                 C.c_void_p, C.c_void_p, C.c_void_p, C.c_void_p, C.c_void_p, C.c_void_p]),
    "ccdm_csscore": (C.c_int, [C.c_void_p, C.c_int64, C.c_void_p, C.c_int, C.c_int, C.c_int, C.c_int, C.c_int, C.c_int, C.c_void_p, C.c_void_p,
                               C.c_void_p, C.c_int, C.c_void_p, C.c_void_p, C.c_void_p, C.c_int, C.c_int, C.c_void_p, C.c_void_p, C.c_void_p,
                               C.c_void_p, C.c_void_p]),
    "ccdm_csscore_ids": (C.c_int, [C.c_void_p, C.c_int, C.c_int, C.c_int, C.c_void_p, C.c_void_p, C.c_int, C.c_void_p, C.c_void_p, C.c_void_p,
                                   C.c_int, C.c_int, C.c_void_p, C.c_void_p, C.c_void_p, C.c_void_p, C.c_void_p]),
    "ccdm_segcalib_workspace_bytes": (C.c_size_t, [C.c_int, C.c_int, C.c_int, C.c_int, C.c_int]),
    "ccdm_segcalib": (C.c_int, [C.c_void_p, C.c_int64, C.c_void_p, C.c_void_p, C.c_int, C.c_int, C.c_int, C.c_int, C.c_int, C.c_int, C.c_int,
                                C.c_void_p, C.c_void_p, C.c_void_p, C.c_void_p, C.c_size_t, C.c_void_p]),
    "ccdm_segboundary_workspace_bytes": (C.c_size_t, [C.c_int, C.c_int, C.c_int]),
    "ccdm_segboundary": (C.c_int, [C.c_void_p, C.c_void_p, C.c_int, C.c_int, C.c_int, C.c_int, C.c_int, C.c_void_p, C.c_void_p, C.c_void_p,
                                   C.c_size_t, C.c_void_p]),
    "ccdm_contourf_workspace_bytes": (C.c_size_t, [C.c_int, C.c_int, C.c_int]),
    "ccdm_contourf": (C.c_int, [C.c_void_p, C.c_void_p, C.c_int, C.c_int, C.c_int, C.c_int, C.c_int, C.c_void_p, C.c_void_p, C.c_size_t,
                                C.c_void_p]),
    "ccdm_uncscore_workspace_bytes": (C.c_size_t, [C.c_int, C.c_int, C.c_int, C.c_int, C.c_int, C.c_int]),
    "ccdm_uncscore": (C.c_int, [C.c_void_p, C.c_int64, C.c_void_p, C.c_void_p, C.c_void_p, C.c_void_p, C.c_int, C.c_int, C.c_int, C.c_int,
                                C.c_int, C.c_int, C.c_int, C.c_int, C.c_int, C.c_void_p, C.c_void_p, C.c_void_p, C.c_size_t, C.c_void_p]),
    "ccdm_attention_ex": (C.c_int, [C.c_void_p, C.c_void_p, C.c_int, C.c_int, C.c_int, C.c_int, C.c_int, C.c_int, C.c_void_p]),
    "ccdm_layernorm": (C.c_int, [C.c_void_p, C.c_void_p, C.c_void_p, C.c_float, C.c_long, C.c_int, C.c_void_p, C.c_void_p]),
    "ccdm_gelu": (C.c_int, [C.c_void_p, C.c_size_t, C.c_void_p, C.c_void_p]),
    "ccdm_vit_key_resize": (C.c_int, [C.c_void_p, C.c_int, C.c_int, C.c_int, C.c_int, C.c_int, C.c_int, C.c_int, C.c_int, C.c_void_p,
                                      C.c_void_p]),
    "ccdm_mix_uniform": (C.c_int, [C.c_void_p, C.c_void_p, C.c_int, C.c_int, C.c_int, C.c_void_p, C.c_void_p]),
    "ccdm_theta_post": (C.c_int, [C.c_void_p, C.c_void_p, C.c_void_p, C.c_void_p, C.c_int, C.c_int, C.c_int, C.c_int, C.c_void_p, C.c_void_p]),
    "ccdm_kl_clamped": (C.c_int, [C.c_void_p, C.c_void_p, C.c_size_t, C.c_float, C.c_void_p, C.c_void_p]),
    "ccdm_nchw_to_nhwc": (C.c_int, [C.c_void_p, C.c_void_p, C.c_int, C.c_int, C.c_int, C.c_int, C.c_int, C.c_void_p]),
    "ccdm_onehot_to_xin": (C.c_int, [C.c_void_p, C.c_void_p, C.c_int, C.c_int, C.c_int, C.c_int, C.c_void_p]),
    "ccdm_engine_create": (C.c_void_p, [C.c_void_p]),
    "ccdm_engine_destroy": (None, [C.c_void_p]),
    "ccdm_engine_add_conv": (C.c_int, [C.c_void_p, C.POINTER(ConvArgs)]),
    "ccdm_engine_add_attention": (C.c_int, [C.c_void_p, C.c_void_p, C.c_void_p, C.c_int, C.c_int, C.c_int, C.c_int, C.c_int]),
    "ccdm_engine_set_epilogue": (C.c_int, [C.c_void_p, C.POINTER(PostArgs)]),
    "ccdm_engine_num_ops": (C.c_int, [C.c_void_p]),
    "ccdm_engine_num_captures": (C.c_int, [C.c_void_p]),
    "ccdm_engine_set_run_block": (C.c_int, [C.c_void_p, C.c_void_p]),
    "ccdm_engine_set_run": (C.c_int, [C.c_void_p, C.c_void_p, C.c_int64, C.c_int32, C.c_uint64, C.c_uint32, C.c_void_p, C.c_void_p, C.c_void_p]),
    "ccdm_engine_run": (C.c_int, [C.c_void_p, C.c_int, C.c_int, C.c_int, C.c_int, C.c_void_p]),
    "ccdm_engine_profile_op": (C.c_int, [C.c_void_p, C.c_int, C.c_int]),
    "ccdm_engine_profile_read": (C.c_int, [C.c_void_p, C.c_int, C.POINTER(C.c_double), C.POINTER(C.c_double), C.POINTER(C.c_double)]),
    "ccdm_engine_describe_op": (C.c_int, [C.c_void_p, C.c_int, C.c_char_p, C.c_int]),
}

_lib: Optional[C.CDLL] = None


class CcdmHipError(RuntimeError):
    pass


class CcdmRangeError(CcdmHipError):
    """The network output of a run was not finite: with PREC_F16X3 the signature of a staged activation beyond the fp16
    split's range (|a| >= 4094, include/ccdm_hip.h).  Outputs of that run are invalid."""


def build(force: bool = False, verbose: bool = False) -> str:
    from concurrent.futures import ThreadPoolExecutor
    srcs = [os.path.join(CSRC, s) for s in SOURCES]
    hdrs = [os.path.join(CSRC, h) for h in sorted(os.listdir(CSRC)) if h.endswith(".h")] + [os.path.join(ROOT, "include", "ccdm_hip.h")]
    objdir = os.path.join(_HERE, "build", "obj")
    os.makedirs(objdir, exist_ok=True)
    wanted = {os.path.basename(s) + ".o" for s in srcs}
    for f in os.listdir(objdir):
        if f.endswith(".o") and f not in wanted:
            os.remove(os.path.join(objdir, f))
    newest_hdr = max(os.path.getmtime(h) for h in hdrs)
    flags = [f for f in HIPCC_FLAGS if f != "-shared"]

    def compile_one(src: str):
        obj = os.path.join(objdir, os.path.basename(src) + ".o")
        if not force and os.path.exists(obj) and os.path.getmtime(obj) >= max(os.path.getmtime(src), newest_hdr):
            return obj, False
        cmd = ["hipcc", *flags, "-I" + os.path.join(ROOT, "include"), "-c", src, "-o", obj]
        if verbose:
            print(" ".join(cmd))
        r = subprocess.run(cmd, capture_output=True, text=True)
        if r.returncode != 0:
            raise CcdmHipError("hipcc failed:\n" + r.stdout + r.stderr)
        return obj, True

    with ThreadPoolExecutor(max_workers=min(len(srcs), os.cpu_count() or 1)) as ex:
        res = list(ex.map(compile_one, srcs))
    objs = [o for o, _ in res]
    if not force and not any(c for _, c in res) and os.path.exists(LIB_PATH) and \
            all(os.path.getmtime(LIB_PATH) >= os.path.getmtime(o) for o in objs):
        return LIB_PATH
    cmd = ["hipcc", "--offload-arch=gfx950", "-shared", "-fPIC", *objs, "-o", LIB_PATH]
    if verbose:
        print(" ".join(cmd))
    r = subprocess.run(cmd, capture_output=True, text=True)
    if r.returncode != 0:
        raise CcdmHipError("hipcc link failed:\n" + r.stdout + r.stderr)
    return LIB_PATH


def load() -> C.CDLL:
    global _lib
    if _lib is not None:
        return _lib
    if not os.path.exists(LIB_PATH):
        import shutil
        if shutil.which("hipcc") and os.path.isdir(CSRC) and not os.environ.get("CCDM_NO_AUTOBUILD"):
            build(force=True)
    if not os.path.exists(LIB_PATH):
        raise CcdmHipError(
            f"{LIB_PATH} not found: the HIP extension is required (no CPU fallback). "
            "Build it with `python -c 'import __graft_entry__ as g; g.build()'`.")
    lib = C.CDLL(LIB_PATH)
    for name, (res, args) in SIGNATURES.items():
        try:
            fn = getattr(lib, name)
        except AttributeError as e:
            raise CcdmHipError(f"{LIB_PATH} does not export {name}") from e
        fn.restype = res
        fn.argtypes = args
    if lib.ccdm_version() != ABI_VERSION:
        raise CcdmHipError(f"{LIB_PATH} implements ABI version {lib.ccdm_version()}, this host code needs {ABI_VERSION}: rebuild it")
    _lib = lib
    return lib


def last_error() -> str:
    return load().ccdm_last_error_string().decode("utf-8", "replace")

# ... 79 lines not shown
```

### ccdm_stochastic_segmentation_amd/models.py

```python
from __future__ import annotations

import logging
import math
from typing import Any, Callable, Dict, List, Mapping, Optional, Sequence, Tuple, Union, cast

import numpy as np
import torch
from torch import Tensor, nn

from . import guidance as G
from . import hip
from .engine import SamplerEngine, TileCanvas
from .guidance import GUIDANCE_KEYWORDS, KNOWN_FREE, VIEW_FLIPS, Guidance, resample_walk, tile_origins
from .unet_spec import UNetSpec, make_unet_spec

LOGGER = logging.getLogger(__name__)

__all__ = ["build_model", "DiffusionModel", "DenoisingModel", "UNetModel", "OneHotCategoricalBCHW",
           "linear_schedule", "cosine_schedule", "step_values", "resample_walk", "pass_key",
           "bound_timesteps", "bound_prior", "bound_rows"]


def linear_schedule(time_steps: int, start=1e-2, end=0.2) -> Tuple[Tensor, Tensor, Tensor]:
    betas = torch.linspace(start, end, time_steps)
# ... 192 lines not shown
        hip.check(lib.ccdm_mix_uniform(x.data_ptr(), s.data_ptr(), N, K, H * W, out.data_ptr(),
                                       torch.cuda.current_stream(x.device).cuda_stream), "mix_uniform")
        return out

    def q_xt_given_xtm1(self, xtm1: Tensor, t: Tensor) -> OneHotCategoricalBCHW:
        s = 1.0 - self._per_sample(self.betas, t, xtm1.shape[0], xtm1.device)
        return OneHotCategoricalBCHW(self._mix(xtm1, s.contiguous()))

    def q_xt_given_x0(self, x0: Tensor, t: Tensor) -> OneHotCategoricalBCHW:
        return OneHotCategoricalBCHW(self._mix(x0, self._per_sample(self.cumalphas, t, x0.shape[0], x0.device)))

    def _theta(self, xt: Tensor, other: Tensor, t: Tensor, prob_mode: int) -> Tensor:
        xt, other = self._dev(xt, "theta_post"), self._dev(other, "theta_post")
        N, K, H, W = xt.shape
        if other.shape != xt.shape:
            raise ValueError(f"theta_post: shapes differ {tuple(xt.shape)} vs {tuple(other.shape)}")
        a, c = self._coeffs(t, N, xt.device)
        out = torch.empty_like(xt)
        lib = hip.load()
        hip.check(lib.ccdm_theta_post(xt.data_ptr(), other.data_ptr(), a.data_ptr(), c.data_ptr(), N, K, H * W, prob_mode,
                                      out.data_ptr(), torch.cuda.current_stream(xt.device).cuda_stream), "theta_post")
        return out

    def theta_post(self, xt: Tensor, x0: Tensor, t: Tensor) -> Tensor:
        return self._theta(xt, x0, t, 0)

    def theta_post_prob(self, xt: Tensor, theta_x0: Tensor, t: Tensor) -> Tensor:
        return self._theta(xt, theta_x0, t, 1)

    def kl_clamped(self, prob_true: Tensor, prob_pred: Tensor, floor: float = 1e-12) -> Tensor:
        p, q = self._dev(prob_true, "kl_clamped"), self._dev(prob_pred, "kl_clamped")
        if p.shape != q.shape:
            raise ValueError(f"kl_clamped: shapes differ {tuple(p.shape)} vs {tuple(q.shape)}")
        out = torch.empty_like(p)
        hip.check(hip.load().ccdm_kl_clamped(p.data_ptr(), q.data_ptr(), p.numel(), float(floor), out.data_ptr(),
                                             torch.cuda.current_stream(p.device).cuda_stream), "kl_clamped")
        return out


class UNetModel(nn.Module):

    def __init__(self, spec: UNetSpec):
        super().__init__()
        self.spec = spec
        self.in_channels, self.model_channels, self.out_channels = spec.in_channels, spec.model_channels, spec.out_channels
        self._version_seen = 0
        self._weights_version = 0

        def container_for(path: List[str]) -> nn.Module:
            mod: nn.Module = self
            for part in path:
                if not hasattr(mod, part):
                    mod.add_module(part, nn.Module())
                mod = getattr(mod, part)
            return mod

        for key, shape in spec.param_shapes().items():
            *path, leaf = key.split(".")
            container_for(path).register_parameter(leaf, nn.Parameter(torch.zeros(shape), requires_grad=False))
        self.register_load_state_dict_post_hook(lambda module, incompatible: module.mark_weights_changed())

    def mark_weights_changed(self) -> None:
        self._weights_version += 1

    def _apply(self, fn, *a, **k):
        r = super()._apply(fn, *a, **k)
        self._weights_version += 1
        return r

    def forward(self, *args, **kwargs):
        raise RuntimeError("UNetModel has no eager forward; call it through DenoisingModel (HIP engine)")


HOST_NOISE_BLOCK_BYTES = 256 << 20


def auto_substreams(N: int, H: int, W: int) -> int:
    return 2 if (N >= 2 and N * H * W >= 32 * 128 * 128) else 1


class DenoisingModel(nn.Module):

    VIEW_FLIPS, KNOWN_FREE = VIEW_FLIPS, KNOWN_FREE

    def __init__(self, diffusion: DiffusionModel, unet: UNetModel, dataset_file: str, step_T_sample: str = "majority"):
        super().__init__()
        self.diffusion = diffusion
        self.unet = unet
        self.dataset_file = dataset_file
        self.step_T_sample = step_T_sample
        self.rng = "philox"
        self.philox_seed = 0
        self.philox_call = 0
        self.philox_advance = True
        self.bound_call = 0
        self.sample_offset = 0
        self.noise_slice: Optional[Tuple[int, int]] = None
        self.use_graph = True
        self.substreams = 0
        self.calibrate_mode = True
        self.mode_choice: Dict[Any, dict] = {}
        self.last_mode: Optional[Tuple[int, bool]] = None
        self.prec = hip.PREC_F16X3
        self.on_range_error = "layers"
        self.f32_layers: set = set()
        self._auto_pins: set = set()
        self._auto_f32_from: Optional[int] = None
        self._auto_weights_key: Optional[Tuple[int, int]] = None
        self.range_events = {"overflows": 0, "layers_pinned": 0, "switched_to_f32": 0, "reset_on_new_weights": 0}
        self._range_probe: Optional[Dict[str, float]] = None
        self.slicing = "throughput"
        self._engines: Dict[Any, Tuple[int, SamplerEngine]] = {}

    @property
    def time_steps(self) -> int:
        return self.diffusion.time_steps

    def _fine_slices(self, N: int) -> int:
        if self.slicing not in ("throughput", "latency"):
            raise ValueError(f"slicing: {self.slicing!r} (expected 'throughput' or 'latency')")
        return 0 if self.slicing != "latency" else (2 if N <= 8 else 1)

    def forward(self, x: Tensor, condition: Tensor, feature_condition: Tensor = None, t: Optional[Tensor] = None,
                label_ref_logits: Optional[Tensor] = None, validation: bool = False, *,
                known_labels: Optional[Tensor] = None, resample: Optional[Tuple[int, int]] = None,
                evidence: Optional[Tensor] = None, temperature: Optional[float] = None,
                truncation: Optional[float] = None, views: Optional[Sequence[str]] = None,
                tiles: Optional[Sequence[int]] = None) -> Union[Tensor, dict]:
        guidance = dict(known_labels=known_labels, resample=resample, evidence=evidence, temperature=temperature, truncation=truncation,
                        views=views, tiles=tiles)
        if self.training or validation:
            G.refuse_outside_sampling(self, guidance)
        if self.training:
            if not isinstance(t, Tensor):
                raise ValueError("'t' needs to be a Tensor at training time")
            if not isinstance(x, Tensor):
                raise ValueError("'x' needs to be a Tensor at training time")
            return self.forward_step(x, condition, feature_condition, t)
        if validation:
            return self.forward_step(x, condition, feature_condition, t)
        return self.forward_denoising(x, condition, feature_condition, None if t is None else cast(int, t.item()), label_ref_logits, **guidance)

    def _weights_key(self) -> Tuple[int, int]:
        return self.unet._weights_version, sum(int(p._version) for p in self.unet.parameters())

    def _engine(self, x: Tensor, condition: Tensor, feature_condition: Optional[Tensor], slot: Any = 0) -> SamplerEngine:
        N, K, H, W = x.shape
        spec = self.unet.spec
        if feature_condition is not None and spec.feature_condition_unwired:
            raise RuntimeError(f"feature_condition given, but input block(s) {spec.feature_condition_unwired} were not widened for it "
                               "(feature_cond_encoder target_layer / output_stride do not line up): channel mismatch")
        fshape = tuple(feature_condition.shape[1:]) if feature_condition is not None else None
        if not spec.feature_condition_idx:
            fshape = None
        dev = next(self.unet.parameters()).device
        f32_layers = frozenset(self.f32_layers) if self.prec == hip.PREC_F16X3 else frozenset()
        key = (N, H, W, int(condition.shape[1]), fshape, str(dev), self.prec, slot, self._fine_slices(N), f32_layers)
        wkey = self._weights_key()
        hit = self._engines.get(key)
        if hit is not None and hit[0] == wkey:
            return hit[1]
        eng = SamplerEngine(spec, self.unet.state_dict(), N, H, W, K, int(condition.shape[1]), dev,
                            max_steps=self.time_steps, feature_shape=fshape, prec=self.prec, fine_slices=self._fine_slices(N),
                            f32_layers=f32_layers)
        self._engines = {k: v for k, v in self._engines.items() if v[0] == wkey}
        self._engines[key] = (wkey, eng)
        return eng

    def sampling_queue(self, capacity: int, image_shape: Sequence[int], guided: bool = False):
        from .serving import SamplingQueue
        return SamplingQueue(self, capacity, image_shape, guided=guided)

    def _philox_key(self, call: Optional[int] = None) -> int:
        call = int(self.philox_call if call is None else call)
        if call == 0:
            return int(self.philox_seed) & 0xFFFFFFFFFFFFFFFF
        z = (int(self.philox_seed) + 0x9E3779B97F4A7C15 * call) & 0xFFFFFFFFFFFFFFFF
        z = ((z ^ (z >> 30)) * 0xBF58476D1CE4E5B9) & 0xFFFFFFFFFFFFFFFF
        z = ((z ^ (z >> 27)) * 0x94D049BB133111EB) & 0xFFFFFFFFFFFFFFFF
        return z ^ (z >> 31)

    @staticmethod
    def _to_index(x: Tensor, device) -> Tensor:
        return x.argmax(dim=1).to(device=device, dtype=torch.uint8).contiguous()

    RANGE_MARGIN = 0.5

    def _probe_ranges(self, engines) -> None:
        if self._range_probe is None:
            return
        for eng in engines:
            hit = self._range_probe.get(id(eng))
            if hit is None:
                hit = self._range_probe[id(eng)] = (eng, eng.probe_buffer())
            eng.probe_ranges(hit[1])

    def _collect_probe(self) -> Optional[Dict[str, float]]:
        if self._range_probe is None:
            return None
        out: Dict[str, float] = {}
        for eng, buf in self._range_probe.values():
            for name, v in eng.read_ranges(buf).items():
                out[name] = max(out.get(name, 0.0), v)
        return out

    def _with_range_fallback(self, fn):
        if self.on_range_error not in ("layers", "f32", "raise"):
            raise ValueError(f"on_range_error: {self.on_range_error!r} (expected 'layers', 'f32' or 'raise')")
        state = torch.get_rng_state() if self.rng == "torch_cpu" else None
        if self._auto_weights_key is not None and self._auto_weights_key != self._weights_key():
            self.f32_layers -= self._auto_pins
            if self._auto_f32_from is not None and self.prec == hip.PREC_F32:
                self.prec = self._auto_f32_from
            self._auto_pins, self._auto_f32_from, self._auto_weights_key = set(), None, None
            self.range_events["reset_on_new_weights"] += 1
        try:
            return fn()
        except hip.CcdmRangeError as e:
            if self.prec == hip.PREC_F32 or self.on_range_error == "raise":
                raise
            self.range_events["overflows"] += 1
            LOGGER.warning("%s -- repeating this call with the exact-fp32 kernels", e)
            if state is not None:
                torch.set_rng_state(state)
            prec, self.prec = self.prec, hip.PREC_F32
            self._range_probe = {} if self.on_range_error == "layers" else None
            probe = None
            try:
                out = fn()
                probe = self._collect_probe()
            finally:
                self.prec = prec
                self._range_probe = None
            if probe is not None:
                limit = hip.F16X3_LIMIT * self.RANGE_MARGIN
                hot = sorted(k for k, v in probe.items() if not (v < limit))
                new = [k for k in hot if k not in self.f32_layers]
                if new:
                    self.f32_layers.update(new)
                    self._auto_pins.update(new)
                    self._auto_weights_key = self._weights_key()
                    self.range_events["layers_pinned"] += len(new)
                    LOGGER.warning("F16X3 range: %d layer(s) stage values beyond %.0f (%s ...); they run the exact-fp32 kernels from now on "
                                   "(DenoisingModel.f32_layers)", len(new), limit, ", ".join(new[:4]))
                    self._engines.clear()
                else:
                    LOGGER.warning("F16X3 range: the overflow could not be attributed to a layer (largest staged value %.3g); this model "
                                   "runs the exact-fp32 kernels until its weights change (DenoisingModel.prec = PREC_F32; range_events counts it)",
                                   max(probe.values()) if probe else float("nan"))
                    self._auto_f32_from, self._auto_weights_key = prec, self._weights_key()
                    self.range_events["switched_to_f32"] += 1
                    self.prec = hip.PREC_F32
                    self._engines = {k: v for k, v in self._engines.items() if k[6] == hip.PREC_F32}
            return out

    CALIBRATION_MIN_STEPS = 100
    CALIBRATION_STEPS = (4, 16)
    CALIBRATION_ROUNDS = 3

    def _calibrate_mode(self, x: Tensor, condition: Tensor, feature_condition: Optional[Tensor], prepare, run_steps,
                        nsub_rule: int, graph_allowed: bool, n_rows: int) -> Tuple[int, bool]:
        import time
        N, K, H, W = x.shape
        ck = (N, K, H, W, int(condition.shape[1]), None if feature_condition is None else tuple(feature_condition.shape[1:]), self.prec,
              self._fine_slices(N), graph_allowed, nsub_rule, self._weights_key())
        hit = self.mode_choice.get(ck)
        if hit is not None:
            return hit["nsub"], hit["use_graph"]
        warm, timed = (max(1, min(int(v), n_rows)) for v in self.CALIBRATION_STEPS)
        cands = [(ns, g) for ns in (nsub_rule, 1) for g in ((True, False) if graph_allowed else (False,))]
        try:
            parts_of = {ns: prepare(ns) for ns in (nsub_rule, 1)}
        except torch.cuda.OutOfMemoryError:
            LOGGER.warning("execution-mode measurement skipped for N=%d %dx%d: no memory for both engine sets; static rule (%d streams)", N, H, W, nsub_rule)
            self._engines = {}
            torch.cuda.empty_cache()
            self.mode_choice[ck] = {"nsub": nsub_rule, "use_graph": graph_allowed, "ms_per_denoise_step": {}}
            return nsub_rule, graph_allowed
        dev = parts_of[1][0][0].device
        for ns, g in cands:
            run_steps(parts_of[ns], 0, warm, [None] * ns, 0, g)
        torch.cuda.synchronize(dev)
        times = {c: float("inf") for c in cands}
        for _ in range(self.CALIBRATION_ROUNDS):
            for ns, g in cands:
                t0 = time.perf_counter()
                run_steps(parts_of[ns], 0, timed, [None] * ns, 0, g)
                torch.cuda.synchronize(dev)
                times[(ns, g)] = min(times[(ns, g)], (time.perf_counter() - t0) / timed * 1e3)
        for parts_ in parts_of.values():
            for eng, lo, hi in parts_:
                eng.check_and_clear_flag()
        best = min(times, key=times.get)
        self.mode_choice = {k_: v for k_, v in self.mode_choice.items() if k_[-1] == ck[-1]}
        self.mode_choice[ck] = {"nsub": best[0], "use_graph": best[1],
                                "ms_per_denoise_step": {f"{ns} stream{'s' if ns > 1 else ''}, {'graph' if g else 'eager'}": round(v, 4) for (ns, g), v in times.items()}}
        LOGGER.info("execution mode for N=%d %dx%d: %d stream(s), %s (ms per denoise step: %s)", N, H, W, best[0], "graph" if best[1] else "eager",
                    self.mode_choice[ck]["ms_per_denoise_step"])
        return best

    def forward_step(self, x: Tensor, condition: Tensor, feature_condition: Tensor, t: Tensor) -> dict:
        return self._with_range_fallback(lambda: self._forward_step(x, condition, feature_condition, t))

    def forward_denoising(self, x: Optional[Tensor], condition: Tensor, feature_condition: Tensor,
                          init_t: Optional[int] = None, label_ref_logits: Optional[Tensor] = None, *,
                          consume: Optional[Callable[[SamplerEngine, int, int], None]] = None,
                          known_labels: Optional[Tensor] = None, resample: Optional[Tuple[int, int]] = None,
                          evidence: Optional[Tensor] = None, temperature: Optional[float] = None,
                          truncation: Optional[float] = None, views: Optional[Sequence[str]] = None,
                          tiles: Optional[Sequence[int]] = None) -> dict:
        guidance = dict(known_labels=known_labels, resample=resample, evidence=evidence, temperature=temperature, truncation=truncation,
                        views=views, tiles=tiles)
        guide = G.check_guidance(self, guidance, None if x is None else tuple(x.shape), feature_condition)
        return self._sample(x, condition, feature_condition, init_t, label_ref_logits, consume, guide)

    def _sample(self, x: Optional[Tensor], condition: Tensor, feature_condition: Tensor, init_t: Optional[int],
                label_ref_logits: Optional[Tensor], consume, guide: Guidance) -> dict:
        out = self._with_range_fallback(lambda: self._forward_denoising(x, condition, feature_condition, init_t, label_ref_logits,
                                                                        consume, guide))
        if self.philox_advance:
            self.philox_call += 1
        return out

    MULTI_MAPS = ("mean", "vote", "entropy", "mutual_info", "counts")

    @torch.no_grad()
    def predict_multiple(self, condition: Tensor, feature_condition: Optional[Tensor] = None, *, num_evaluations: int,
                         voting: Optional[str] = None, x: Optional[Tensor] = None, t: Optional[Tensor] = None, batched: bool = False,
                         maps: Sequence[str] = ("mean", "vote", "entropy", "mutual_info"),
                         known_labels: Optional[Tensor] = None, resample: Optional[Tuple[int, int]] = None,
                         evidence: Optional[Tensor] = None, temperature: Optional[float] = None,
                         truncation: Optional[float] = None, views: Optional[Sequence[str]] = None,
                         tiles: Optional[Sequence[int]] = None) -> Dict[str, Tensor]:
        voting = self.step_T_sample if voting is None else voting
        if voting not in ("confidence", "majority"):
            raise ValueError(f"voting: {voting!r} (expected 'confidence' or 'majority')")
        if isinstance(num_evaluations, bool) or int(num_evaluations) != num_evaluations or int(num_evaluations) < 1:
            raise ValueError(f"num_evaluations: {num_evaluations!r} (expected an integer >= 1)")
        S = int(num_evaluations)
        maps = tuple(maps)
        bad = [m for m in maps if m not in self.MULTI_MAPS or (m == "counts" and voting != "majority")]
        if bad:
            raise ValueError(f"maps: {bad} not available (choose from {self.MULTI_MAPS}; 'counts' with voting='majority')")
        guidance = dict(known_labels=known_labels, resample=resample, evidence=evidence, temperature=temperature, truncation=truncation,
                        views=views, tiles=tiles)
        init_t, guide, batch = self._samples_per_image(condition, feature_condition, S, x, t, guidance, interleaved=batched)
        B, H, W = int(condition.shape[0]), int(condition.shape[2]), int(condition.shape[3])
        K, HW = self.diffusion.num_classes, H * W
# ... 270 lines not shown
        eng = self._engine(x, condition, feature_condition)
        N = x.shape[0]
        tt = t.detach().float().reshape(-1).cpu()
        if tt.numel() == 1:
            tt = tt.expand(N)
        with eng.enter():
            eng.set_inputs(self._to_index(x, eng.device), condition.to(eng.device), feature_condition)
            eng.set_tables([float(v) for v in tt], [(0.0, 1.0, hip.STEP_SOFTMAX_ONLY)] * N, per_sample=True)
            eng.run(1, with_epilogue=True, use_graph=False)
            out = eng.out_probs.clone().permute(0, 3, 1, 2)
            logits = eng.ce_logits()
        eng.leave()
        eng.raise_if_flagged()
        self._probe_ranges([eng])
        return {"diffusion_out": out, "logits": logits}

    def _forward_denoising(self, x: Optional[Tensor], condition: Tensor, feature_condition: Tensor,
                           init_t: Optional[int] = None, label_ref_logits: Optional[Tensor] = None, consume=None,
                           guide: Guidance = Guidance()) -> dict:
        known, evidence, shaping, views, tiles = guide.known, guide.evidence, guide.shaping, guide.views, guide.tiles
        V = 1 if views is None else 1 + len(views)
        if label_ref_logits is not None:
            raise AttributeError("'DenoisingModel' object has no attribute 'guidance_scale_weights'")
        T = self.time_steps
        t_values = step_values(T, init_t)
        N, K, H, W = x.shape
        S = len(t_values)
        vote = self.step_T_sample
        last_mode = (hip.STEP_LAST_MAJORITY if vote is None or vote == "majority"
                     else hip.STEP_LAST_CONFIDENCE if vote == "confidence" else hip.STEP_LAST_KEEP)
        coeffs = []
        for t in t_values:
            a, c = self.diffusion.posterior_coeffs(t)
            coeffs.append((a, c, hip.STEP_SAMPLE if t > 1 else last_mode))
        if self.rng not in ("philox", "torch_cpu"):
            raise ValueError(f"unknown rng mode {self.rng!r}")
        host_rng = self.rng == "torch_cpu"
        stop_at_x0 = evidence is not None or shaping is not None or views is not None or tiles is not None
        oys, oxs = tile_origins(H, W, *tiles) if tiles is not None else ([0], [0])
        R = len(oys) * len(oxs)
        canvases: Dict[int, TileCanvas] = {}
        table = coeffs if not stop_at_x0 else [(a_, c_, hip.STEP_SOFTMAX_ONLY) for a_, c_, m_ in coeffs]
        clamp_c = [1.0 if j == S - 1 else c_ for j, (a_, c_, m_) in enumerate(coeffs)]
        key = self._philox_key()
        walk = guide.walk(S)
        renoise_p: Dict[int, Tuple[float, float]] = {}
        cum = self.diffusion.cumalphas.detach().cpu().double() if len(walk) > S else None
        for e, (row, _, src) in enumerate(walk):
            if src is not None:
                r_ = float(cum[t_values[row] - 1]) / float(cum[t_values[src] - 1])
                p_move = (1.0 - r_) / K
                renoise_p[e] = (float(np.float32(r_ + p_move)), float(np.float32(p_move)))
        gN, first = self.noise_slice if (host_rng and self.noise_slice is not None) else (N, 0)
        def mirrored(a: Tensor) -> Tensor:
            return torch.cat([a] + [torch.flip(a, [d for b, d in ((1, 3), (2, 2)) if f & b]) for f in cast(tuple, views)], 0)

        def tiled(a: Tensor) -> Tensor:
            h_, w_ = cast(tuple, tiles)[:2]
            return torch.cat([a[:, :, oy:oy + h_, ox:ox + w_] for oy in oys for ox in oxs], 0)

        rows = tiled if tiles is not None else None if views is None else mirrored
        fc_axis = G.sample_axis(feature_condition, views, tiles)

        def prepare(nsub_: int):
            bounds = [(N * j) // nsub_ for j in range(nsub_ + 1)]
            parts_ = []
            for j in range(nsub_):
                lo, hi = bounds[j], bounds[j + 1]
                xs, cs = (x[lo:hi], condition[lo:hi]) if rows is None else (rows(x[lo:hi]), rows(condition[lo:hi]))
                fc = None
                if feature_condition is not None and (rows is None or self.unet.spec.feature_condition_idx):
                    fc = feature_condition.narrow(fc_axis, lo, hi - lo)
                    fc = fc.flatten(0, 1) if fc_axis == 1 else fc
                eng = self._engine(xs, cs, fc, slot=j)
                with eng.enter():
                    eng.set_inputs(self._to_index(xs, eng.device), cs.to(eng.device), fc)
                    eng.set_tables([float(t) for t in t_values], table)
                    if tiles is not None:
                        canvases[lo] = eng.tile_canvas(hi - lo, H, W, tiles[2], tiles[3])
                        canvases[lo].xt.copy_(self._to_index(x[lo:hi], eng.device).reshape(hi - lo, H * W))
                parts_.append((eng, lo, hi))
            return parts_

        def run_row(eng, lo: int, hi: int, row: int, kp: int, renoise, noise, noise_row0_: int, graph_: bool):
            off = self.sample_offset + lo
            if renoise is not None:
                eng.renoise(*renoise, row, philox_seed=kp, sample_offset=off)
            eng.run(1, first_row=row, noise=noise, noise_row0=noise_row0_, philox_seed=kp, sample_offset=off, use_graph=graph_)
            if stop_at_x0:
                eng.guided_step(None if evidence is None else evidence[lo:hi], shaping, views, *coeffs[row], row, philox_seed=kp, sample_offset=off,
                                canvas=canvases.get(lo))
            if known is not None:
                eng.clamp_known_labels(known[lo:hi], clamp_c[row], coeffs[row][2], row, philox_seed=kp, sample_offset=off)

        def run_steps(parts_, s0_: int, s1_: int, noises_, noise_row0_: int, graph_: bool):
            if len(parts_) == 1 and not guide:
                parts_[0][0].run(s1_ - s0_, first_row=s0_, noise=noises_[0], noise_row0=noise_row0_, philox_seed=key,
                                 sample_offset=self.sample_offset, use_graph=graph_)
                return
            for e in range(s0_, s1_):
                row, p, _ = walk[e]
                for j, (eng, lo, hi) in enumerate(parts_):
                    run_row(eng, lo, hi, row, pass_key(key, p), renoise_p.get(e), noises_[j], noise_row0_, graph_)

        nsub = int(self.substreams) if int(self.substreams) > 0 else (
            auto_substreams(V * N, H, W) if tiles is None else auto_substreams(R * N, tiles[0], tiles[1]))
        nsub = max(1, min(nsub, N))
        use_graph = bool(self.use_graph)
        if (int(self.substreams) <= 0 and self.calibrate_mode and not host_rng and self._range_probe is None and nsub > 1
                and S >= self.CALIBRATION_MIN_STEPS and not guide):
            nsub, use_graph = self._calibrate_mode(x, condition, feature_condition, prepare, run_steps, nsub, use_graph, S)
        self.last_mode = (nsub, use_graph)
        parts = prepare(nsub)
        if host_rng:
            per_step = gN * H * W * K * 4
            blk = max(1, HOST_NOISE_BLOCK_BYTES // max(per_step, 1))
            blocks = [(s0, min(s0 + blk, S)) for s0 in range(0, S, blk)]
        else:
            blocks = [(0, len(walk))]
        if self._range_probe is not None:
            blocks = [(s, s + 1) for s in range(len(walk))]
        for s0, s1 in blocks:
            noises: List[Optional[Tensor]] = [None] * nsub
            if host_rng:
                host = torch.empty((s1 - s0, gN, H * W * K), dtype=torch.float32)
                for j in range(s0, s1):
                    if t_values[j] > 1:
                        host[j - s0].view(-1).exponential_(1)
                for j, (eng, lo, hi) in enumerate(parts):
                    with torch.cuda.stream(eng.stream):
                        noises[j] = host[:, first + lo:first + hi].contiguous().to(eng.device)
            run_steps(parts, s0, s1, noises, s0, use_graph)
            self._probe_ranges([p_[0] for p_ in parts])
        outs = []
        for eng, lo, hi in (parts if consume is None else []):
            with eng.enter():
                n_ = hi - lo
                src = canvases.get(lo, eng)
                if t_values[-1] > 1 or last_mode == hip.STEP_LAST_KEEP:
                    idx = src.xt.reshape(-1, H, W)[:n_].long()
                    out = torch.nn.functional.one_hot(idx, K).permute(0, 3, 1, 2).to(torch.float32)
                elif last_mode == hip.STEP_LAST_CONFIDENCE:
                    out = src.out_probs[:n_].clone().permute(0, 3, 1, 2)
                else:
                    out = src.out_onehot[:n_].clone().permute(0, 3, 1, 2)
            eng.leave()
            outs.append(out)
        flagged = [eng.check_and_clear_flag() for eng, lo, hi in parts]
        if any(flagged):
            parts[0][0].raise_range_error()
        if consume is not None:
            for eng, lo, hi in parts:
                with eng.enter():
                    consume(canvases.get(lo, eng), lo, hi)
                eng.leave()
            return {}
        out = outs[0] if nsub == 1 else torch.cat(outs, 0)
        if out.device != x.device:
            out = out.to(x.device)
        return {"diffusion_out": out}


def build_model(
        time_steps: int,
        schedule: str,
        schedule_params: Union[dict, None],
        input_shapes: List[Tuple[int, int, int]],
        cond_encoded_shape,
        backbone: str,
        backbone_params: Dict[str, Any],
        dataset_file: str,
        step_T_sample: str = None,
        feature_cond_encoder: dict = None
) -> DenoisingModel:
    img_shape, label_shape = input_shapes
    img_channels = img_shape[0]
    num_classes = label_shape[0]
    if not 2 <= num_classes <= hip.MAX_CLASSES:
        raise ValueError(f"label shape {tuple(label_shape)}: {num_classes} classes, the HIP sampler is built for 2..{hip.MAX_CLASSES} (DESIGN.md section 8)")
    diffusion = DiffusionModel(schedule, time_steps, num_classes, schedule_params=schedule_params)
    if backbone == "unet_openai":
        spec = make_unet_spec(
            image_size=min(img_shape[1], img_shape[2]),
            in_channels=num_classes + img_channels,
            out_channels=num_classes,
            num_res_blocks=2,
# ... 10 lines not shown
```

### include/ccdm_hip.h

```cpp
#ifndef CCDM_HIP_H
#define CCDM_HIP_H

#include <stddef.h>
#include <stdint.h>

#ifdef __cplusplus
extern "C" {
#endif

#define CCDM_ABI_VERSION 11
#define CCDM_MAX_CHANNELS 1024
#define CCDM_STATS_MAX_SLICES 64
#define CCDM_STATS_FOLD_SLICES 16

int ccdm_version(void);
const char* ccdm_last_error_string(void);

int ccdm_gn_stats(const float* x , int N, int HW, int C, int slices,
                  double* stats , void* stream);

enum { CCDM_ACT_NONE = 0, CCDM_ACT_SILU = 1 };
enum { CCDM_PREC_F32 = 0,
       CCDM_PREC_F16X3 = 1,
       CCDM_PREC_F16 = 2 };
// ... 258 lines not shown
                     int L, const uint8_t* ignore_in_eval, const uint8_t* category, const uint8_t* has_instances, int inst_base, int NI,
                     int64_t* conf, int64_t* per_image, int32_t* instances, int32_t* unknown, void* stream);

size_t ccdm_segcalib_workspace_bytes(int B, int H, int W, int K, int M);
int ccdm_segcalib(const float* probs , int64_t pixel_stride, const uint8_t* cls ,
                  const uint8_t* labels , int B, int h, int w, int H, int W, int K, int M,
                  int64_t* bins , double* conf_sum , double* sums , void* workspace,
                  size_t workspace_bytes, void* stream);

size_t ccdm_segboundary_workspace_bytes(int B, int H, int W);
int ccdm_segboundary(const uint8_t* pred , const uint8_t* labels , int B, int H, int W,
                     int K, int d, int64_t* bcounts , int64_t* trimap , void* workspace,
                     size_t workspace_bytes, void* stream);

size_t ccdm_contourf_workspace_bytes(int B, int H, int W);
int ccdm_contourf(const uint8_t* pred , const uint8_t* labels , int B, int H, int W, int K,
                  int theta, int64_t* counts , void* workspace, size_t workspace_bytes, void* stream);

size_t ccdm_uncscore_workspace_bytes(int B, int H, int W, int K, int U, int M);
int ccdm_uncscore(const float* probs , int64_t pixel_stride, const uint8_t* cls ,
                  const uint8_t* labels , const float* maps , const float* ranges ,
                  int B, int h, int w, int H, int W, int K, int U, int M, int P, int64_t* pix ,
                  int64_t* patch , void* workspace, size_t workspace_bytes, void* stream);

int ccdm_vote_accumulate(const uint8_t* cls , const float* probs , int64_t src_stride,
                         int B, int HW, int K, float w, float* total ,
                         int32_t* counts , float* ent_sum , void* stream);
int ccdm_vote_finalize(const float* total , const int32_t* counts ,
                       const float* ent_sum , int B, int HW, int K, int S,
                       float* mean , uint8_t* vote ,
                       float* entropy , float* mutual_info , void* stream);
int ccdm_vote_reduce_stack(const uint8_t* stack , int B, int S, int HW, int K,
                           int32_t* counts , float* mean ,
                           uint8_t* vote , float* entropy , void* stream);

int ccdm_modes_distance(const uint8_t* a , int B, int S, int HW, int K, int32_t* ws ,
                        int32_t* Q , void* stream);
int ccdm_modes_pam(const int32_t* Q , int B, int S, int M, int max_swaps, int32_t* medoid ,
                   int32_t* assign , int32_t* size , int64_t* spread , int64_t* cost ,
                   int32_t* swaps , int32_t* converged , void* stream);
int ccdm_modes_maps(const uint8_t* a , const int32_t* assign , const int32_t* size , int B, int S,
                    int M, int HW, int K, uint8_t* vote , int32_t* counts ,
                    float* entropy , void* stream);

int ccdm_mix_uniform(const float* x , const float* s, int N, int K, int HW, float* out, void* stream);
int ccdm_theta_post(const float* xt , const float* x0 , const float* a, const float* c,
                    int N, int K, int HW, int prob_mode, float* out , void* stream);
int ccdm_kl_clamped(const float* p, const float* q, size_t n, float floor, float* out, void* stream);

int ccdm_attention_ex(const float* qkv , float* out , int N, int T, int T_alloc, int C,
                      int heads, int order, void* stream);
int ccdm_layernorm(const float* x, const float* gamma, const float* beta, float eps, long rows, int C, float* out, void* stream);
int ccdm_gelu(const float* x, size_t n, float* out, void* stream);
int ccdm_vit_key_resize(const float* qkv , int N, int T_alloc, int h0, int w0, int dim, int heads, int Ht, int Wt,
                        float* out , void* stream);

int ccdm_nchw_to_nhwc(const float* src, float* dst, int N, int C, int HW, int dst_stride, int dst_off, void* stream);
int ccdm_onehot_to_xin(const uint8_t* idx, float* xin, int N, int HW, int K, int xin_stride, void* stream);

typedef struct ccdm_engine ccdm_engine;

ccdm_engine* ccdm_engine_create(int32_t* step_counter );
void ccdm_engine_destroy(ccdm_engine* e);
int ccdm_engine_add_conv(ccdm_engine* e, const ccdm_conv_args* a);
int ccdm_engine_add_attention(ccdm_engine* e, const float* qkv, float* out, int N, int T, int C, int heads, int order);
int ccdm_engine_add_norm_qkv_attention(ccdm_engine* e, const ccdm_attn_block_args* a);
int ccdm_engine_add_stats_fold(ccdm_engine* e, const double* in, int N, int S_in, int C, int S_out, double* out);
int ccdm_engine_add_resample(ccdm_engine* e, const ccdm_resample_args* a);
int ccdm_engine_add_stem(ccdm_engine* e, const ccdm_stem_args* a);
int ccdm_engine_add_head_posterior(ccdm_engine* e, const ccdm_head_args* a);
int ccdm_engine_set_epilogue(ccdm_engine* e, const ccdm_post_args* a);
int ccdm_engine_num_ops(const ccdm_engine* e);
int ccdm_engine_num_captures(const ccdm_engine* e);
int ccdm_engine_set_run_block(ccdm_engine* e, void* dev_block);
int ccdm_engine_set_run(ccdm_engine* e, const float* noise, int64_t noise_step_stride, int32_t noise_row0,
                        uint64_t philox_seed, uint32_t sample_offset,
                        float* out_probs, int64_t* out_onehot, float* posterior_out);
int ccdm_engine_run(ccdm_engine* e, int first_row, int n_steps, int with_epilogue, int use_graph, void* stream);
int ccdm_engine_profile_op(ccdm_engine* e, int op_index, int capacity);
int ccdm_engine_profile_read(ccdm_engine* e, int op_index, double* mean_ms, double* min_ms, double* max_ms);
int ccdm_engine_input_absmax(ccdm_engine* e, float* out, int row, void* stream);
int ccdm_engine_describe_op(const ccdm_engine* e, int i, char* buf, int buflen);

#ifdef __cplusplus
}
#endif
#endif
```

Baseline: 91.93.

## Fork low-resolution UNet ops into per-sample-range branches on side streams

Adds row-range views for the conv, attention, stats-fold and resample ops, and an engine fork. The fork splits the longest run of low-resolution ops by batch samples into two branches that launch on separate streams, joined by events and captured into a separate graph. The goal is to fill the GPU during small-spatial layers, where a single launch covers too few tiles. The cost is more kernel launches and event waits per step, and each branch runs at a smaller batch, which lowers per-kernel efficiency.

```diff
diff --git a/ccdm_stochastic_segmentation_amd/csrc/ccdm_attn_block.hip b/ccdm_stochastic_segmentation_amd/csrc/ccdm_attn_block.hip
--- a/ccdm_stochastic_segmentation_amd/csrc/ccdm_attn_block.hip
+++ b/ccdm_stochastic_segmentation_amd/csrc/ccdm_attn_block.hip
@@ -277,6 +277,23 @@
     return 0;
 }
 
+ccdm_attn_block_args attn_block_rows(const ccdm_attn_block_args& a, int n0, int n) {
+    ccdm_attn_block_args r = a;
+    const size_t k = (size_t)n0;
+    r.N = n;
+    r.x = rows_advance(a.x, k * a.T * a.C);
+    r.stats = rows_advance(a.stats, k * a.slices * a.C * 2);
+    r.out = rows_advance(a.out, k * a.T * a.C);
+    return r;
+}
+
+}
+
+extern "C" int ccdm_norm_qkv_attention_rows(const ccdm_attn_block_args* a, int n0, int n, ccdm_attn_block_args* out) {
+    CCDM_REQUIRE(a && out, "ccdm_norm_qkv_attention_rows: null args");
+    CCDM_REQUIRE(n0 >= 0 && n >= 1 && n0 <= a->N - n, "ccdm_norm_qkv_attention_rows: rows [%d, %d + %d) of %d", n0, n0, n, a->N);
+    *out = ccdm::attn_block_rows(*a, n0, n);
+    return 0;
 }
 
 extern "C" int ccdm_norm_qkv_attention_supported(int T, int C, int heads) { return ccdm::attn_block_supported(T, C, heads) ? 1 : 0; }
diff --git a/ccdm_stochastic_segmentation_amd/csrc/ccdm_common.h b/ccdm_stochastic_segmentation_amd/csrc/ccdm_common.h
--- a/ccdm_stochastic_segmentation_amd/csrc/ccdm_common.h
+++ b/ccdm_stochastic_segmentation_amd/csrc/ccdm_common.h
@@ -79,4 +79,12 @@
 int launch_head(const ccdm_head_args& a, const ccdm_post_args& post, hipStream_t s);
 bool attn_block_supported(int T, int C, int heads);
 
+ccdm_conv_args conv_rows(const ccdm_conv_args& a, int n0, int n);
+ccdm_attn_block_args attn_block_rows(const ccdm_attn_block_args& a, int n0, int n);
+ccdm_resample_args resample_rows(const ccdm_resample_args& a, int n0, int n);
+void attention_rows(const float*& qkv, float*& out, int& N, int T, int C, int n0, int n);
+void stats_fold_rows(const double*& in, double*& out, int& N, int S_in, int C, int S_out, int n0, int n);
+template <typename T>
+static inline T* rows_advance(T* p, size_t k) { return p ? p + k : p; }
+
 }
diff --git a/ccdm_stochastic_segmentation_amd/csrc/ccdm_conv.hip b/ccdm_stochastic_segmentation_amd/csrc/ccdm_conv.hip
--- a/ccdm_stochastic_segmentation_amd/csrc/ccdm_conv.hip
+++ b/ccdm_stochastic_segmentation_amd/csrc/ccdm_conv.hip
@@ -958,6 +958,30 @@
     return 0;
 }
 
+ccdm_conv_args conv_rows(const ccdm_conv_args& a, int n0, int n) {
+    ccdm_conv_args r = a;
+    const size_t k = (size_t)n0, in_px = (size_t)a.Hin * a.Win, out_px = (size_t)a.Hout * a.Wout;
+    r.N = n;
+    r.in0 = rows_advance(a.in0, k * in_px * a.C0);
+    r.in1 = rows_advance(a.in1, k * in_px * a.C1);
+    r.stats0 = rows_advance(a.stats0, k * a.slices0 * a.C0 * 2);
+    r.stats1 = rows_advance(a.stats1, k * a.slices1 * a.C1 * 2);
+    r.emb_row_of_sample = rows_advance(a.emb_row_of_sample, k);
+    r.resid = rows_advance(a.resid, k * out_px * a.Cout);
+    r.out = rows_advance(a.out, k * out_px * a.Cout);
+    r.out_stats = rows_advance(a.out_stats, k * a.out_slices * a.Cout * 2);
+    r.skip0 = rows_advance(a.skip0, k * out_px * a.SC0);
+    r.skip1 = rows_advance(a.skip1, k * out_px * a.SC1);
+    return r;
+}
+
+}
+
+extern "C" int ccdm_conv_rows(const ccdm_conv_args* a, int n0, int n, ccdm_conv_args* out) {
+    CCDM_REQUIRE(a && out, "ccdm_conv_rows: null args");
+    CCDM_REQUIRE(n0 >= 0 && n >= 1 && n0 <= a->N - n, "ccdm_conv_rows: rows [%d, %d + %d) of %d", n0, n0, n, a->N);
+    *out = ccdm::conv_rows(*a, n0, n);
+    return 0;
 }
 
 extern "C" int ccdm_conv_slices(int Hout, int Wout, int stride, int ksize) {
diff --git a/ccdm_stochastic_segmentation_amd/csrc/ccdm_engine.hip b/ccdm_stochastic_segmentation_amd/csrc/ccdm_engine.hip
--- a/ccdm_stochastic_segmentation_amd/csrc/ccdm_engine.hip
+++ b/ccdm_stochastic_segmentation_amd/csrc/ccdm_engine.hip
@@ -45,6 +45,27 @@
     }
 }
 
+static bool op_rows(const Op& op, int n0, int n, Op& r) {
+    r = op;
+    switch (op.kind) {
+        case 0: r.conv = conv_rows(op.conv, n0, n); return true;
+        case 1: attention_rows(r.qkv, r.out, r.N, op.T, op.C, n0, n); return true;
+        case 2: stats_fold_rows(r.fin, r.fout, r.N, op.S_in, op.C, op.S_out, n0, n); return true;
+        case 3: r.ab = attn_block_rows(op.ab, n0, n); return true;
+        case 4: r.rs = resample_rows(op.rs, n0, n); return true;
+        default: return false;
+    }
+}
+static int op_batch(const Op& op) {
+    switch (op.kind) {
+        case 0: return op.conv.N;
+        case 1: case 2: return op.N;
+        case 3: return op.ab.N;
+        case 4: return op.rs.N;
+        default: return -1;
+    }
+}
+
 }
 
 struct ccdm_engine {
@@ -56,25 +77,55 @@
     ccdm_post_run* run_dev = nullptr;
     bool run_dirty = false;
     int next_row = 0;
-    hipGraph_t graph = nullptr;
-    hipGraphExec_t exec = nullptr;
-    bool graph_valid = false;
-    int graph_with_epilogue = -1;
+    hipGraph_t graph[2] = {nullptr, nullptr};
+    hipGraphExec_t exec[2] = {nullptr, nullptr};
+    bool graph_valid[2] = {false, false};
+    int graph_with_epilogue[2] = {-1, -1};
     int captures = 0;
     struct Tap { std::vector<hipEvent_t> ev; int n = 0; };
     std::map<int, Tap> taps;
+    int fork_first = -1, fork_last = -1;
+    std::vector<std::vector<ccdm::Op>> fork_ops;
+    std::vector<hipStream_t> side;
+    hipEvent_t fork_ev = nullptr;
+    std::vector<hipEvent_t> join_ev;
+    bool fork_on = true;
+    int64_t forked_steps = 0;
 };
 
 using namespace ccdm;
 
-static void drop_graph(ccdm_engine* e) {
-    if (e->exec) { (void)hipGraphExecDestroy(e->exec); e->exec = nullptr; }
-    if (e->graph) { (void)hipGraphDestroy(e->graph); e->graph = nullptr; }
-    e->graph_valid = false;
-}
-
-static int launch_step(ccdm_engine* e, int with_epilogue, hipStream_t s, bool profile) {
+static void drop_graph(ccdm_engine* e, int g) {
+    if (e->exec[g]) { (void)hipGraphExecDestroy(e->exec[g]); e->exec[g] = nullptr; }
+    if (e->graph[g]) { (void)hipGraphDestroy(e->graph[g]); e->graph[g] = nullptr; }
+    e->graph_valid[g] = false;
+}
+static void drop_graph(ccdm_engine* e) { drop_graph(e, 0); drop_graph(e, 1); }
+
+static int launch_forked(ccdm_engine* e, hipStream_t s) {
+    const size_t B = e->fork_ops.size();
+    if (hipEventRecord(e->fork_ev, s) != hipSuccess) return fail("engine_run: fork event: %s", hipGetErrorString(hipGetLastError()));
+    for (size_t b = 1; b < B; ++b)
+        if (hipStreamWaitEvent(e->side[b - 1], e->fork_ev, 0) != hipSuccess) return fail("engine_run: fork wait: %s", hipGetErrorString(hipGetLastError()));
+    int rc = 0;
+    for (size_t j = 0; j < e->fork_ops[0].size() && !rc; ++j)
+        for (size_t b = 0; b < B && !rc; ++b) rc = launch_op(e->fork_ops[b][j], b ? e->side[b - 1] : s);
+    for (size_t b = 1; b < B; ++b) {
+        if (hipEventRecord(e->join_ev[b - 1], e->side[b - 1]) != hipSuccess || hipStreamWaitEvent(s, e->join_ev[b - 1], 0) != hipSuccess) {
+            if (!rc) rc = fail("engine_run: join: %s", hipGetErrorString(hipGetLastError()));
+        }
+    }
+    return rc;
+}
+
+static int launch_step(ccdm_engine* e, int with_epilogue, hipStream_t s, bool profile, bool forked) {
     for (size_t i = 0; i < e->ops.size(); ++i) {
+        if (forked && (int)i == e->fork_first) {
+            const int rc = launch_forked(e, s);
+            if (rc) return rc;
+            i = (size_t)e->fork_last;
+            continue;
+        }
         const Op& op = e->ops[i];
         ccdm_engine::Tap* tp = nullptr;
         if (profile) {
@@ -105,9 +156,20 @@
     return e;
 }
 
+static void drop_fork(ccdm_engine* e) {
+    e->fork_ops.clear();
+    e->fork_first = e->fork_last = -1;
+    for (hipStream_t st : e->side) (void)hipStreamDestroy(st);
+    e->side.clear();
+    for (hipEvent_t ev : e->join_ev) (void)hipEventDestroy(ev);
+    e->join_ev.clear();
+    if (e->fork_ev) { (void)hipEventDestroy(e->fork_ev); e->fork_ev = nullptr; }
+}
+
 extern "C" void ccdm_engine_destroy(ccdm_engine* e) {
     if (!e) return;
     drop_graph(e);
+    drop_fork(e);
     for (auto& kv : e->taps)
         for (hipEvent_t ev : kv.second.ev) (void)hipEventDestroy(ev);
     delete e;
@@ -201,6 +263,67 @@
     drop_graph(e);
     return 0;
 }
+
+extern "C" int ccdm_engine_set_fork(ccdm_engine* e, int first_op, int last_op, int branches) {
+    CCDM_REQUIRE(e, "engine_set_fork: null engine");
+    CCDM_REQUIRE(branches <= CCDM_ENGINE_MAX_BRANCHES, "engine_set_fork: %d branches (at most %d)", branches, CCDM_ENGINE_MAX_BRANCHES);
+    drop_graph(e);
+    drop_fork(e);
+    if (branches <= 1) return 0;
+    CCDM_REQUIRE(first_op >= 0 && first_op <= last_op && last_op < (int)e->ops.size(), "engine_set_fork: ops %d..%d of %d", first_op, last_op, (int)e->ops.size());
+    const int N = op_batch(e->ops[first_op]);
+    for (int i = first_op; i <= last_op; ++i) {
+        const int n = op_batch(e->ops[i]);
+        if (n < 0) return 0;
+        CCDM_REQUIRE(n == N, "engine_set_fork: op %d runs %d samples, op %d runs %d", i, n, first_op, N);
+    }
+    if (N < 2) return 0;
+    const int B = branches < N ? branches : N;
+    std::vector<std::vector<Op>> fo((size_t)B);
+    for (int b = 0, n0 = 0; b < B; ++b) {
+        const int n = N / B + (b < N % B ? 1 : 0);
+        for (int i = first_op; i <= last_op; ++i) {
+            Op r;
+            if (!op_rows(e->ops[i], n0, n, r)) return fail("engine_set_fork: op %d has no row-range form", i);
+            fo[(size_t)b].push_back(r);
+        }
+        n0 += n;
+    }
+    e->fork_ops.swap(fo);
+    e->fork_first = first_op;
+    e->fork_last = last_op;
+    return 0;
+}
+
+static int ensure_fork_streams(ccdm_engine* e) {
+    if (!e->fork_ev && hipEventCreateWithFlags(&e->fork_ev, hipEventDisableTiming) != hipSuccess) { e->fork_ev = nullptr; return fail("engine_run: hipEventCreate failed"); }
+    while (e->join_ev.size() + 1 < e->fork_ops.size()) {
+        hipStream_t st;
+        hipEvent_t ev;
+        if (e->side.size() == e->join_ev.size()) {
+            if (hipStreamCreateWithFlags(&st, hipStreamNonBlocking) != hipSuccess) return fail("engine_run: hipStreamCreate failed");
+            e->side.push_back(st);
+        }
+        if (hipEventCreateWithFlags(&ev, hipEventDisableTiming) != hipSuccess) return fail("engine_run: hipEventCreate failed");
+        e->join_ev.push_back(ev);
+    }
+    return 0;
+}
+
+extern "C" int ccdm_engine_fork_info(const ccdm_engine* e, int* first_op, int* last_op) {
+    CCDM_REQUIRE(e, "engine_fork_info: null engine");
+    if (first_op) *first_op = e->fork_first;
+    if (last_op) *last_op = e->fork_last;
+    return e->fork_ops.empty() ? 1 : (int)e->fork_ops.size();
+}
+
+extern "C" int ccdm_engine_enable_fork(ccdm_engine* e, int on) {
+    CCDM_REQUIRE(e, "engine_enable_fork: null engine");
+    e->fork_on = on != 0;
+    return 0;
+}
+
+extern "C" int64_t ccdm_engine_num_forked_steps(const ccdm_engine* e) { return e ? e->forked_steps : -1; }
 
 extern "C" int ccdm_engine_num_ops(const ccdm_engine* e) { return e ? (int)e->ops.size() : -1; }
 extern "C" int ccdm_engine_num_captures(const ccdm_engine* e) { return e ? e->captures : -1; }
@@ -256,31 +379,39 @@
         use_graph = 0;
         if (first_row == 0) for (auto& kv : e->taps) kv.second.n = 0;
     }
+    const bool forked = !profile && e->fork_on && !e->fork_ops.empty();
+    if (forked && (!e->fork_ev || e->join_ev.size() + 1 != e->fork_ops.size())) {
+        const int rc = ensure_fork_streams(e);
+        if (rc) return rc;
+    }
     if (use_graph) {
-        if (!e->graph_valid || e->graph_with_epilogue != with_epilogue) {
-            drop_graph(e);
+        const int g = forked ? 1 : 0;
+        if (!e->graph_valid[g] || e->graph_with_epilogue[g] != with_epilogue) {
+            drop_graph(e, g);
             hipError_t err = hipStreamBeginCapture(s, hipStreamCaptureModeRelaxed);
             if (err != hipSuccess) return fail("engine_run: BeginCapture: %s", hipGetErrorString(err));
-            const int rc = launch_step(e, with_epilogue, s, false);
-            err = hipStreamEndCapture(s, &e->graph);
-            if (rc) { if (e->graph) { (void)hipGraphDestroy(e->graph); e->graph = nullptr; } return rc; }
+            const int rc = launch_step(e, with_epilogue, s, false, forked);
+            err = hipStreamEndCapture(s, &e->graph[g]);
+            if (rc) { if (e->graph[g]) { (void)hipGraphDestroy(e->graph[g]); e->graph[g] = nullptr; } return rc; }
             if (err != hipSuccess) return fail("engine_run: EndCapture: %s", hipGetErrorString(err));
-            err = hipGraphInstantiate(&e->exec, e->graph, nullptr, nullptr, 0);
+            err = hipGraphInstantiate(&e->exec[g], e->graph[g], nullptr, nullptr, 0);
             if (err != hipSuccess) return fail("engine_run: GraphInstantiate: %s", hipGetErrorString(err));
-            e->graph_valid = true;
-            e->graph_with_epilogue = with_epilogue;
+            e->graph_valid[g] = true;
+            e->graph_with_epilogue[g] = with_epilogue;
             e->captures++;
         }
         for (int i = 0; i < n_steps; ++i) {
-            hipError_t err = hipGraphLaunch(e->exec, s);
+            hipError_t err = hipGraphLaunch(e->exec[g], s);
             if (err != hipSuccess) return fail("engine_run: GraphLaunch: %s", hipGetErrorString(err));
         }
+        if (forked) e->forked_steps += n_steps;
         return 0;
     }
     for (int i = 0; i < n_steps; ++i) {
-        int rc = launch_step(e, with_epilogue, s, profile);
+        int rc = launch_step(e, with_epilogue, s, profile, forked);
         if (rc) return rc;
     }
+    if (forked) e->forked_steps += n_steps;
     return 0;
 }
 
diff --git a/ccdm_stochastic_segmentation_amd/csrc/ccdm_misc.hip b/ccdm_stochastic_segmentation_amd/csrc/ccdm_misc.hip
--- a/ccdm_stochastic_segmentation_amd/csrc/ccdm_misc.hip
+++ b/ccdm_stochastic_segmentation_amd/csrc/ccdm_misc.hip
@@ -154,6 +154,12 @@
     return 0;
 }
 
+void attention_rows(const float*& qkv, float*& out, int& N, int T, int C, int n0, int n) {
+    qkv = rows_advance(qkv, (size_t)n0 * T * 3 * C);
+    out = rows_advance(out, (size_t)n0 * T * C);
+    N = n;
+}
+
 __device__ __forceinline__ float silu_t(float x) { return x / (1.0f + expf(-x)); }
 
 __global__ void k_time_table(const float* __restrict__ sinus, int mc,
@@ -241,6 +247,11 @@
     hipLaunchKernelGGL(k_stats_fold, grid, dim3(256), 0, s, in, S_in, 2 * C, S_out, out);
     CCDM_CHECK_LAUNCH("stats_fold");
     return 0;
+}
+void stats_fold_rows(const double*& in, double*& out, int& N, int S_in, int C, int S_out, int n0, int n) {
+    in = rows_advance(in, (size_t)n0 * S_in * 2 * C);
+    out = rows_advance(out, (size_t)n0 * S_out * 2 * C);
+    N = n;
 }
 }
 
diff --git a/ccdm_stochastic_segmentation_amd/csrc/ccdm_resample.hip b/ccdm_stochastic_segmentation_amd/csrc/ccdm_resample.hip
--- a/ccdm_stochastic_segmentation_amd/csrc/ccdm_resample.hip
+++ b/ccdm_stochastic_segmentation_amd/csrc/ccdm_resample.hip
@@ -90,6 +90,25 @@
     return 0;
 }
 
+ccdm_resample_args resample_rows(const ccdm_resample_args& a, int n0, int n) {
+    ccdm_resample_args r = a;
+    const size_t k = (size_t)n0, in_px = (size_t)a.Hin * a.Win;
+    const size_t out_px = a.mode == CCDM_RESAMPLE_AVGPOOL2 ? (size_t)(a.Hin / 2) * (a.Win / 2) : 4 * in_px;
+    r.N = n;
+    r.in = rows_advance(a.in, k * in_px * a.C);
+    r.stats = rows_advance(a.stats, k * a.slices * a.C * 2);
+    r.out_act = rows_advance(a.out_act, k * out_px * a.C);
+    r.out_raw = rows_advance(a.out_raw, k * out_px * a.C);
+    return r;
+}
+
+}
+
+extern "C" int ccdm_resample_rows(const ccdm_resample_args* a, int n0, int n, ccdm_resample_args* out) {
+    CCDM_REQUIRE(a && out, "ccdm_resample_rows: null args");
+    CCDM_REQUIRE(n0 >= 0 && n >= 1 && n0 <= a->N - n, "ccdm_resample_rows: rows [%d, %d + %d) of %d", n0, n0, n, a->N);
+    *out = ccdm::resample_rows(*a, n0, n);
+    return 0;
 }
 
 extern "C" int ccdm_resample(const ccdm_resample_args* a, void* stream) {
diff --git a/ccdm_stochastic_segmentation_amd/engine.py b/ccdm_stochastic_segmentation_amd/engine.py
--- a/ccdm_stochastic_segmentation_amd/engine.py
+++ b/ccdm_stochastic_segmentation_amd/engine.py
@@ -54,8 +54,10 @@
     def __init__(self, spec: UNetSpec, state_dict: Dict[str, torch.Tensor], N: int, H: int, W: int,
                  num_classes: int, img_channels: int, device: torch.device, max_steps: int,
                  feature_shape: Optional[Tuple[int, int, int]] = None, prec: int = hip.PREC_F32, fine_slices: int = 0,
-                 f32_layers=frozenset()):
+                 f32_layers=frozenset(), fork_branches: int = 0):
         self.lib = hip.load()
+        self.fork_branches = int(fork_branches)
+        self._fork_on = True
         self.f32_layers = frozenset(f32_layers)
         self.fine_slices = int(fine_slices)
         if device.type != "cuda":
@@ -425,6 +427,7 @@
                                      io_bytes=4 * (h.C * H * W + Kp * H * W), gn_read_bytes=4 * h.C * H * W, weight_bytes=4 * Kp * h.C * 9,
                                      flop=2 * h.C * Kp * 9 * H * W))
         self.n_unet_ops = lib.ccdm_engine_num_ops(self._handle)
+        self._set_fork()
 
         post = hip.PostArgs()
         post.head, post.softmax, post.head_stride = (0 if self.head_fused else self.head.ptr), int(spec.softmax_output), (Kp if self.head_fused else self.head.C)
@@ -444,6 +447,41 @@
         self._sd = None
         self._tables_key = None
         self._per_sample_rows = False
+
+    FORK_MAX_PIXELS = 32 * 32
+    FORK_MAX_BATCH = 96
+
+    def fork_range(self) -> Optional[Tuple[int, int]]:
+        px, low = 0, []
+        for i in range(self.n_unet_ops):
+            info = self.op_info[i]
+            if info["kind"] in ("conv", "resample"):
+                px = info["hout"] * info["wout"]
+            elif info["kind"] in ("attention", "norm_qkv_attention"):
+                px = info["T"]
+            low.append(px <= self.FORK_MAX_PIXELS and not info.get("stem") and not info.get("head_fused"))
+        best, start = None, None
+        for i, ok in enumerate(low + [False]):
+            if ok and start is None:
+                start = i
+            elif not ok and start is not None:
+                if i - start >= 2 and (best is None or i - start > best[1] - best[0] + 1):
+                    best = (start, i - 1)
+                start = None
+        return best
+
+    def _set_fork(self) -> None:
+        rng = self.fork_range()
+        if self.fork_branches > 1 and rng is not None and 2 <= self.N <= self.FORK_MAX_BATCH:
+            hip.check(self.lib.ccdm_engine_set_fork(self._handle, rng[0], rng[1], self.fork_branches), "engine_set_fork")
+
+    def fork_info(self) -> Tuple[int, int, int]:
+        a, b = C.c_int(), C.c_int()
+        n = hip.check(self.lib.ccdm_engine_fork_info(self._handle, C.byref(a), C.byref(b)), "engine_fork_info")
+        return n, a.value, b.value
+
+    def forked_steps(self) -> int:
+        return int(self.lib.ccdm_engine_num_forked_steps(self._handle))
 
     def __del__(self):
         try:
@@ -596,7 +634,10 @@
 
     def run(self, n_steps: int, *, noise: Optional[torch.Tensor] = None, philox_seed: int = 0, sample_offset: int = 0,
             with_epilogue: bool = True, use_graph: bool = False, first_row: int = 0, noise_row0: int = 0,
-            posterior_out: Optional[torch.Tensor] = None) -> None:
+            posterior_out: Optional[torch.Tensor] = None, fork: bool = True) -> None:
+        if bool(fork) != self._fork_on:
+            hip.check(self.lib.ccdm_engine_enable_fork(self._handle, int(bool(fork))), "engine_enable_fork")
+            self._fork_on = bool(fork)
         npn = self.N * self.H * self.W * self.K
         if noise is not None:
             assert noise.is_cuda and noise.dtype == torch.float32 and noise.is_contiguous()
diff --git a/ccdm_stochastic_segmentation_amd/hip.py b/ccdm_stochastic_segmentation_amd/hip.py
--- a/ccdm_stochastic_segmentation_amd/hip.py
+++ b/ccdm_stochastic_segmentation_amd/hip.py
@@ -277,6 +277,13 @@
     "ccdm_engine_profile_op": (C.c_int, [C.c_void_p, C.c_int, C.c_int]),
     "ccdm_engine_profile_read": (C.c_int, [C.c_void_p, C.c_int, C.POINTER(C.c_double), C.POINTER(C.c_double), C.POINTER(C.c_double)]),
     "ccdm_engine_describe_op": (C.c_int, [C.c_void_p, C.c_int, C.c_char_p, C.c_int]),
+    "ccdm_conv_rows": (C.c_int, [C.POINTER(ConvArgs), C.c_int, C.c_int, C.POINTER(ConvArgs)]),
+    "ccdm_norm_qkv_attention_rows": (C.c_int, [C.POINTER(AttnBlockArgs), C.c_int, C.c_int, C.POINTER(AttnBlockArgs)]),
+    "ccdm_resample_rows": (C.c_int, [C.POINTER(ResampleArgs), C.c_int, C.c_int, C.POINTER(ResampleArgs)]),
+    "ccdm_engine_set_fork": (C.c_int, [C.c_void_p, C.c_int, C.c_int, C.c_int]),
+    "ccdm_engine_fork_info": (C.c_int, [C.c_void_p, C.POINTER(C.c_int), C.POINTER(C.c_int)]),
+    "ccdm_engine_enable_fork": (C.c_int, [C.c_void_p, C.c_int]),
+    "ccdm_engine_num_forked_steps": (C.c_int64, [C.c_void_p]),
 }
 
 _lib: Optional[C.CDLL] = None
diff --git a/ccdm_stochastic_segmentation_amd/models.py b/ccdm_stochastic_segmentation_amd/models.py
--- a/ccdm_stochastic_segmentation_amd/models.py
+++ b/ccdm_stochastic_segmentation_amd/models.py
@@ -298,6 +298,10 @@
 class DenoisingModel(nn.Module):
 
     VIEW_FLIPS, KNOWN_FREE = VIEW_FLIPS, KNOWN_FREE
+    fork_lowres = True
+    fork_branches = 2
+    fork_substreams = False
+    fork_eager = False
 
     def __init__(self, diffusion: DiffusionModel, unet: UNetModel, dataset_file: str, step_T_sample: str = "majority"):
         super().__init__()
@@ -371,14 +375,15 @@
             fshape = None
         dev = next(self.unet.parameters()).device
         f32_layers = frozenset(self.f32_layers) if self.prec == hip.PREC_F16X3 else frozenset()
-        key = (N, H, W, int(condition.shape[1]), fshape, str(dev), self.prec, slot, self._fine_slices(N), f32_layers)
+        fork = int(self.fork_branches) if self.fork_lowres else 0
+        key = (N, H, W, int(condition.shape[1]), fshape, str(dev), self.prec, slot, self._fine_slices(N), f32_layers, fork)
         wkey = self._weights_key()
         hit = self._engines.get(key)
         if hit is not None and hit[0] == wkey:
             return hit[1]
         eng = SamplerEngine(spec, self.unet.state_dict(), N, H, W, K, int(condition.shape[1]), dev,
                             max_steps=self.time_steps, feature_shape=fshape, prec=self.prec, fine_slices=self._fine_slices(N),
-                            f32_layers=f32_layers)
+                            f32_layers=f32_layers, fork_branches=fork)
         self._engines = {k: v for k, v in self._engines.items() if v[0] == wkey}
         self._engines[key] = (wkey, eng)
         return eng
@@ -479,7 +484,7 @@
         import time
         N, K, H, W = x.shape
         ck = (N, K, H, W, int(condition.shape[1]), None if feature_condition is None else tuple(feature_condition.shape[1:]), self.prec,
-              self._fine_slices(N), graph_allowed, nsub_rule, self._weights_key())
+              self._fine_slices(N), graph_allowed, nsub_rule, self._weights_key(), int(self.fork_branches) if self.fork_lowres else 0)
         hit = self.mode_choice.get(ck)
         if hit is not None:
             return hit["nsub"], hit["use_graph"]
@@ -916,11 +921,11 @@
                 parts_.append((eng, lo, hi))
             return parts_
 
-        def run_row(eng, lo: int, hi: int, row: int, kp: int, renoise, noise, noise_row0_: int, graph_: bool):
+        def run_row(eng, lo: int, hi: int, row: int, kp: int, renoise, noise, noise_row0_: int, graph_: bool, fork_: bool):
             off = self.sample_offset + lo
             if renoise is not None:
                 eng.renoise(*renoise, row, philox_seed=kp, sample_offset=off)
-            eng.run(1, first_row=row, noise=noise, noise_row0=noise_row0_, philox_seed=kp, sample_offset=off, use_graph=graph_)
+            eng.run(1, first_row=row, noise=noise, noise_row0=noise_row0_, philox_seed=kp, sample_offset=off, use_graph=graph_, fork=fork_)
             if stop_at_x0:
                 eng.guided_step(None if evidence is None else evidence[lo:hi], shaping, views, *coeffs[row], row, philox_seed=kp, sample_offset=off,
                                 canvas=canvases.get(lo))
@@ -928,14 +933,15 @@
                 eng.clamp_known_labels(known[lo:hi], clamp_c[row], coeffs[row][2], row, philox_seed=kp, sample_offset=off)
 
         def run_steps(parts_, s0_: int, s1_: int, noises_, noise_row0_: int, graph_: bool):
+            fork_ = (len(parts_) == 1 or bool(self.fork_substreams)) and (graph_ or bool(self.fork_eager))
             if len(parts_) == 1 and not guide:
                 parts_[0][0].run(s1_ - s0_, first_row=s0_, noise=noises_[0], noise_row0=noise_row0_, philox_seed=key,
-                                 sample_offset=self.sample_offset, use_graph=graph_)
+                                 sample_offset=self.sample_offset, use_graph=graph_, fork=fork_)
                 return
             for e in range(s0_, s1_):
                 row, p, _ = walk[e]
                 for j, (eng, lo, hi) in enumerate(parts_):
-                    run_row(eng, lo, hi, row, pass_key(key, p), renoise_p.get(e), noises_[j], noise_row0_, graph_)
+                    run_row(eng, lo, hi, row, pass_key(key, p), renoise_p.get(e), noises_[j], noise_row0_, graph_, fork_)
 
         nsub = int(self.substreams) if int(self.substreams) > 0 else (
             auto_substreams(V * N, H, W) if tiles is None else auto_substreams(R * N, tiles[0], tiles[1]))
diff --git a/include/ccdm_hip.h b/include/ccdm_hip.h
--- a/include/ccdm_hip.h
+++ b/include/ccdm_hip.h
@@ -364,6 +364,16 @@
 int ccdm_engine_input_absmax(ccdm_engine* e, float* out, int row, void* stream);
 int ccdm_engine_describe_op(const ccdm_engine* e, int i, char* buf, int buflen);
 
+int ccdm_conv_rows(const ccdm_conv_args* a, int n0, int n, ccdm_conv_args* out);
+int ccdm_norm_qkv_attention_rows(const ccdm_attn_block_args* a, int n0, int n, ccdm_attn_block_args* out);
+int ccdm_resample_rows(const ccdm_resample_args* a, int n0, int n, ccdm_resample_args* out);
+
+#define CCDM_ENGINE_MAX_BRANCHES 8
+int ccdm_engine_set_fork(ccdm_engine* e, int first_op, int last_op, int branches);
+int ccdm_engine_fork_info(const ccdm_engine* e, int* first_op, int* last_op);
+int ccdm_engine_enable_fork(ccdm_engine* e, int on);
+int64_t ccdm_engine_num_forked_steps(const ccdm_engine* e);
+
 #ifdef __cplusplus
 }
 #endif
```

Result: no change. 91.23 (-0.8%).
